# BogdanDIA/gr-dvbt

Hardware: AMD Instinct MI355X
Metric: RX Msamples/s (baseband in -> TS out) (higher is better)
Workload: dtype u8 (Viterbi/RS) + f32 (front end)

## Files before the change

gr_dvbt_amd/binding.py:

```python
import ctypes as C
import os
import subprocess
import numpy as np

_HERE = os.path.dirname(os.path.abspath(__file__))
_ROOT = os.path.dirname(_HERE)
_SO = os.path.join(_HERE, "lib", "libdvbt_hip.so")
_SRC = os.path.join(_HERE, "csrc", "dvbt_hip.hip")

QPSK, QAM16, QAM64 = 0, 1, 2
AUTO = -1
NH = 0
C1_2, C2_3, C3_4, C5_6, C7_8 = 0, 1, 2, 3, 4
T2k, T8k = 0, 1
G1_32, G1_16, G1_8, G1_4 = 0, 1, 2, 3
(TAP_ACQ, TAP_FFT, TAP_EQ, TAP_DEMAP, TAP_SYMDEINT, TAP_BITDEINT, TAP_VITERBI, TAP_DEINT, TAP_RS,
 TAP_TS, TAP_CP_START, TAP_SYMBOL_INDEX, TAP_FREQ_OFFSET, TAP_BITDEINT_LP, TAP_SOFT, TAP_CSI, TAP_BITDEINT_LOG) = range(17)
ALPHA1, ALPHA2, ALPHA4 = 1, 2, 3


class DvbtError(RuntimeError):
    pass


# ... 165 lines not shown
    def set_cut(self, stream_symbol_offset):
        cut = RxCut(int(stream_symbol_offset), 0, 0)
        _chk(self.L.dvbt_rx_set_cut(self.h, C.byref(cut)))

    def run_device(self, dptr, nsamples, stream=None):
        rep = RxReport()
        _chk(self.L.dvbt_rx_segment_run_device(self.h, C.c_void_p(dptr), nsamples, C.c_void_p(stream) if stream else None, C.byref(rep)))
        self.report = rep
        return rep

    def enqueue_device(self, dptr, nsamples, stream=None):
        _chk(self.L.dvbt_rx_segment_enqueue_device(self.h, C.c_void_p(dptr), nsamples,
                                                   C.c_void_p(stream) if stream else None))

    def finish(self):
        rep = RxReport()
        _chk(self.L.dvbt_rx_segment_finish(self.h, C.byref(rep)))
        self.report = rep
        return rep

    def tap(self, tap):
        r = self.report
        d = self.dims
        sizes = {TAP_ACQ: r.n_symbols * d.fft_length * 8, TAP_FFT: r.n_symbols * d.fft_length * 8,
                 TAP_EQ: r.n_out_symbols * d.payload_length * 8, TAP_DEMAP: r.n_out_symbols * d.payload_length,
                 TAP_SYMDEINT: r.n_out_symbols * d.payload_length, TAP_BITDEINT: r.n_out_symbols * d.payload_length,
                 TAP_VITERBI: r.n_viterbi_bytes, TAP_DEINT: r.n_rs_bytes // 188 * 204, TAP_RS: r.n_rs_bytes,
                 TAP_TS: r.n_ts_bytes, TAP_CP_START: r.n_symbols * 4, TAP_SYMBOL_INDEX: max(r.n_symbols - 1, 0) * 4,
                 TAP_FREQ_OFFSET: max(r.n_symbols - 1, 0) * 4, TAP_BITDEINT_LP: r.n_out_symbols * d.payload_length,
                 TAP_SOFT: r.n_out_symbols * d.payload_length * d.m, TAP_CSI: r.n_out_symbols * d.payload_length * 4}
        nbytes = max(int(sizes[tap]), 0)
        buf = np.zeros(nbytes, np.uint8)
        if nbytes:
            n = _chk(self.L.dvbt_rx_read_tap(self.h, tap, buf.ctypes.data_as(C.c_void_p), nbytes))
            buf = buf[:n]
        out = buf.view(self._TAP_DTYPE.get(tap, np.uint8))
        if tap in (TAP_ACQ, TAP_FFT):
            out = out.reshape(-1, d.fft_length)
        elif tap in (TAP_EQ, TAP_DEMAP, TAP_SYMDEINT, TAP_BITDEINT, TAP_BITDEINT_LP, TAP_CSI):
            out = out.reshape(-1, d.payload_length)
        elif tap == TAP_SOFT:
            out = out.reshape(-1, d.payload_length * d.m)
        return out

    def lock_periods(self):
        n = _chk(self.L.dvbt_rx_lock_periods(self.h, None, 0))
        buf = (LockPeriod * max(n, 1))()
        _chk(self.L.dvbt_rx_lock_periods(self.h, buf, n))
        return [(b.offset, b.first_call, b.cp_start0, b.n_symbols, b.first_out_symbol) for b in buf[:n]]

    def walk_stats(self):
        class W(C.Structure):
            _fields_ = [("small_passes", C.c_int64), ("general_passes", C.c_int64), ("small_chunk_calls", C.c_int32), ("small_max_calls", C.c_int32)]
        w = W()
        self.L.dvbt_rx_walk_stats.argtypes = [C.c_void_p, C.POINTER(W)]
        _chk(self.L.dvbt_rx_walk_stats(self.h, C.byref(w)))
        return w.small_passes, w.general_passes, w.small_chunk_calls, w.small_max_calls

    def period_taps(self):
        class P(C.Structure):
            _fields_ = [("bitdeint_offset", C.c_int64), ("bitdeint_bytes", C.c_int64), ("viterbi_offset", C.c_int64), ("viterbi_bytes", C.c_int64)]
        self.L.dvbt_rx_period_taps.argtypes = [C.c_void_p, C.c_void_p, C.c_int]
        n = _chk(self.L.dvbt_rx_period_taps(self.h, None, 0))
        buf = (P * max(n, 1))()
        _chk(self.L.dvbt_rx_period_taps(self.h, buf, n))
        total = max([b.bitdeint_offset + b.bitdeint_bytes for b in buf[:n]] + [0])
        log = np.zeros(total, np.uint8)
        if total:
            _chk(self.L.dvbt_rx_read_tap(self.h, TAP_BITDEINT_LOG, log.ctypes.data_as(C.c_void_p), total))
        return [(log[b.bitdeint_offset:b.bitdeint_offset + b.bitdeint_bytes], int(b.viterbi_offset), int(b.viterbi_bytes)) for b in buf[:n]]

    def viterbi_proof(self):
        p = ViterbiProof()
        self.L.dvbt_rx_viterbi_proof.argtypes = [C.c_void_p, C.POINTER(ViterbiProof)]
        _chk(self.L.dvbt_rx_viterbi_proof(self.h, C.byref(p)))
        return {"chunks": int(p.chunks), "decoded_again": int(p.decoded_again), "sequential": int(p.sequential), "not_proven": int(p.not_proven)}

    def viterbi_proof_total(self):
        p = ViterbiProof()
        self.L.dvbt_rx_viterbi_proof_total.argtypes = [C.c_void_p, C.POINTER(ViterbiProof)]
        _chk(self.L.dvbt_rx_viterbi_proof_total(self.h, C.byref(p)))
        return {"chunks": int(p.chunks), "decoded_again": int(p.decoded_again), "sequential": int(p.sequential), "not_proven": int(p.not_proven)}

    def viterbi_check(self):
        a, b = C.c_int64(), C.c_int64()
        self.L.dvbt_rx_viterbi_check.argtypes = [C.c_void_p, C.POINTER(C.c_int64), C.POINTER(C.c_int64)]
        _chk(self.L.dvbt_rx_viterbi_check(self.h, C.byref(a), C.byref(b)))
        return int(a.value), int(b.value)

    def tap_device_ptr(self, tap):
        return self.L.dvbt_rx_tap_device_ptr(self.h, tap)

    def enable_timing(self, on=True):
        _chk(self.L.dvbt_rx_enable_timing(self.h, int(on)))

    def stage_ms(self, name):
        return self.L.dvbt_rx_stage_ms(self.h, name.encode())

    def close(self):
        if self.h:
            self.L.dvbt_rx_destroy(self.h)
            self.h = C.c_void_p()

    def __del__(self):
        try:
            self.close()
        except Exception:
            pass


class StreamParams(C.Structure):
    _fields_ = [("rx", RxParams), ("segment_superframes", C.c_int), ("rank", C.c_int), ("world", C.c_int), ("ts_ring_bytes", C.c_int64), ("borrow_device_pushes", C.c_int), ("chains", C.c_int)]


class StreamInfo(C.Structure):
    _fields_ = [("status", C.c_int32), ("pieces_in_flight", C.c_int32), ("finished", C.c_int32),
                ("samples_pushed", C.c_int64), ("ts_bytes_decoded", C.c_int64), ("ts_bytes_ready", C.c_int64), ("ts_bytes_pulled", C.c_int64),
                ("first_superframe_call", C.c_int64), ("first_ts_packet", C.c_int64),
                ("constellation", C.c_int32), ("hierarchy", C.c_int32), ("code_rate", C.c_int32), ("auto_configured", C.c_int32), ("samples_released", C.c_int64), ("in_walk", C.c_int32)]


class RxStream:

    def __init__(self, constellation, code_rate, mode, segment_superframes=0, guard=G1_32, hierarchy=NH, snr_db=30.0, viterbi_bsize=768,
                 rs_oracle_compat=0, device=0, rank=0, world=0, soft_decision=0, ts_ring_bytes=0, borrow=0, viterbi_warm_windows=0, viterbi_verify=0, chains=0):
        self.L = lib()
        for fn in ("create", "push", "push_device", "finish", "status"):
            getattr(self.L, f"dvbt_rx_stream_{fn}").restype = C.c_int
        self.L.dvbt_rx_stream_create.argtypes = [C.POINTER(StreamParams), C.POINTER(C.c_void_p)]
        self.L.dvbt_rx_stream_push.argtypes = [C.c_void_p, C.c_void_p, C.c_size_t]
        self.L.dvbt_rx_stream_push_device.argtypes = [C.c_void_p, C.c_void_p, C.c_size_t, C.c_void_p]
        self.L.dvbt_rx_stream_pull.restype = C.c_int64
        self.L.dvbt_rx_stream_pull.argtypes = [C.c_void_p, C.c_void_p, C.c_size_t]
        self.L.dvbt_rx_stream_finish.argtypes = [C.c_void_p]
        self.L.dvbt_rx_stream_status.argtypes = [C.c_void_p, C.POINTER(StreamInfo)]
        self.L.dvbt_rx_stream_destroy.argtypes = [C.c_void_p]
        rx = RxParams(constellation, hierarchy, code_rate, guard, mode, 0, 0, snr_db, viterbi_bsize, rs_oracle_compat, 1, 0, device, 0, 0, 0, 0.0, soft_decision)
        rx.viterbi_warm_windows = viterbi_warm_windows
        rx.viterbi_verify = viterbi_verify
        self.p = StreamParams(rx, segment_superframes, rank, world, ts_ring_bytes, borrow, chains)
        self.L.dvbt_rx_stream_pull_chunk.restype = C.c_int64
        self.L.dvbt_rx_stream_pull_chunk.argtypes = [C.c_void_p, C.c_void_p, C.c_size_t, C.POINTER(C.c_int64)]
        self.h = C.c_void_p()
        _chk(self.L.dvbt_rx_stream_create(C.byref(self.p), C.byref(self.h)))
        self._out = np.empty(1 << 22, np.uint8)

    def push(self, iq):
        iq = np.ascontiguousarray(iq, dtype=np.complex64)
        _chk(self.L.dvbt_rx_stream_push(self.h, iq.ctypes.data_as(C.c_void_p), len(iq)))

    def push_device(self, dptr, nsamples, stream=None):
        _chk(self.L.dvbt_rx_stream_push_device(self.h, C.c_void_p(dptr), nsamples, C.c_void_p(stream) if stream else None))

    def pull(self, max_bytes=None):
        chunks = []
        left = max_bytes
        while left is None or left > 0:
            cap = len(self._out) if left is None else min(len(self._out), left)
            n = _chk(self.L.dvbt_rx_stream_pull(self.h, self._out.ctypes.data_as(C.c_void_p), cap))
            if n <= 0:
                break
            chunks.append(self._out[:n].copy())
            if left is not None:
                left -= n
        return np.concatenate(chunks) if chunks else np.zeros(0, np.uint8)

# ... 191 lines not shown
TAG_SYNC_START, TAG_SUPERFRAME_START, TAG_SYMBOL_INDEX = 1, 2, 3


class Tag(C.Structure):
    _fields_ = [("rel_offset", C.c_int64), ("key", C.c_int32), ("value", C.c_int32)]


class Sideband(C.Structure):
    _fields_ = [("in_tags", C.POINTER(Tag)), ("n_in_tags", C.c_int), ("out_tags", C.POINTER(Tag)), ("out_cap", C.c_int),
                ("n_out_tags", C.c_int), ("n_consumed", C.c_int)]


def _params(fields):
    return type("P", (C.Structure,), {"_fields_": fields})


_I = C.c_int
BLOCK_PARAMS = {
    "ofdm_sym_acquisition": _params([("blocks", _I), ("fft_length", _I), ("occupied_tones", _I), ("cp_length", _I), ("snr", C.c_float)]),
    "fft": _params([("fft_size", _I), ("forward", _I), ("shift", _I)]),
    "demod_reference_signals": _params([(n, _I) for n in ("itemsize", "ninput", "noutput", "constellation", "hierarchy", "code_rate_hp",
                                                          "code_rate_lp", "guard_interval", "transmission_mode", "include_cell_id", "cell_id")]),
    "demap": _params([("nsize", _I), ("constellation", _I), ("hierarchy", _I), ("transmission_mode", _I), ("gain", C.c_float)]),
    "symbol_inner_interleaver": _params([("nsize", _I), ("transmission_mode", _I), ("direction", _I)]),
    "bit_inner_deinterleaver": _params([("nsize", _I), ("constellation", _I), ("hierarchy", _I), ("transmission_mode", _I)]),
    "viterbi_decoder": _params([("constellation", _I), ("hierarchy", _I), ("code_rate", _I), ("bsize", _I), ("S0", _I), ("SK", _I)]),
    "convolutional_deinterleaver": _params([("blocks", _I), ("I", _I), ("M", _I)]),
    "reed_solomon_dec": _params([(n, _I) for n in ("p", "m", "gfpoly", "n", "k", "t", "s", "blocks", "oracle_compat")]),
    "energy_descramble": _params([("nblocks", _I)]),
    "resampler": _params([("interpolation", _I), ("decimation", _I), ("scale", C.c_float)]),
    "energy_dispersal": _params([("nblocks", _I)]),
    "reed_solomon_enc": _params([(n, _I) for n in ("p", "m", "gfpoly", "n", "k", "t", "s", "blocks")]),
    "convolutional_interleaver": _params([("blocks", _I), ("I", _I), ("M", _I)]),
    "inner_coder": _params([(n, _I) for n in ("ninput", "noutput", "constellation", "hierarchy", "code_rate")]),
    "bit_inner_interleaver": _params([("nsize", _I), ("constellation", _I), ("hierarchy", _I), ("transmission_mode", _I)]),
    "map": _params([("nsize", _I), ("constellation", _I), ("hierarchy", _I), ("transmission_mode", _I), ("gain", C.c_float)]),
    "reference_signals": _params([(n, _I) for n in ("itemsize", "ninput", "noutput", "constellation", "hierarchy", "code_rate_hp",
                                                    "code_rate_lp", "guard_interval", "transmission_mode", "include_cell_id", "cell_id")]),
}
TX_BLOCKS = ("energy_dispersal", "reed_solomon_enc", "convolutional_interleaver", "inner_coder", "bit_inner_interleaver", "map", "reference_signals")


class Block:

    def __init__(self, name, *args):
        self.L = lib()
        self.name = name
        self.params = BLOCK_PARAMS[name](*args)
        self.h = C.c_void_p()
        _chk(getattr(self.L, f"dvbt_{name}_create")(C.byref(self.params), C.byref(self.h)))
        self._work = getattr(self.L, f"dvbt_{name}_work")
        self._work.argtypes = [C.c_void_p, C.c_int, C.c_int, C.c_void_p, C.c_void_p, C.POINTER(Sideband)]
        self._work_device = getattr(self.L, f"dvbt_{name}_work_device", None)
        if self._work_device is not None:
            self._work_device.argtypes = [C.c_void_p, C.c_int, C.c_int, C.c_void_p, C.c_void_p, C.POINTER(Sideband), C.c_void_p]
        self._tout = (Tag * 4096)()

    def forecast(self, noutput_items):
        n = C.c_int()
        _chk(getattr(self.L, f"dvbt_{self.name}_forecast")(self.h, noutput_items, C.byref(n)))
        return n.value

    def work(self, noutput_items, ninput_items, inp, out, tags=()):
        tin = (Tag * max(len(tags), 1))(*[Tag(*t) for t in tags])
        tout = (Tag * 4096)()
        sb = Sideband(tin, len(tags), tout, 4096, 0, 0)
        r = _chk(self._work(self.h, noutput_items, ninput_items, inp.ctypes.data_as(C.c_void_p), out.ctypes.data_as(C.c_void_p), C.byref(sb)))
        return r, sb.n_consumed, [(tout[i].rel_offset, tout[i].key, tout[i].value) for i in range(min(sb.n_out_tags, 4096))]

    def work_device(self, noutput_items, ninput_items, in_ptr, out_ptr, tags=(), stream=None):
        tin = (Tag * max(len(tags), 1))(*[Tag(*t) for t in tags])
        tout = self._tout
        sb = Sideband(tin, len(tags), tout, 4096, 0, 0)
        r = _chk(self._work_device(self.h, noutput_items, ninput_items, C.c_void_p(in_ptr), C.c_void_p(out_ptr), C.byref(sb),
                                   C.c_void_p(stream) if stream else None))
        return r, sb.n_consumed, [(tout[i].rel_offset, tout[i].key, tout[i].value) for i in range(min(sb.n_out_tags, 4096))]

    def viterbi_proof(self):
        p = ViterbiProof()
        self.L.dvbt_viterbi_decoder_proof.argtypes = [C.c_void_p, C.POINTER(ViterbiProof)]
        _chk(self.L.dvbt_viterbi_decoder_proof(self.h, C.byref(p)))
        return {"chunks": int(p.chunks), "decoded_again": int(p.decoded_again), "sequential": int(p.sequential), "not_proven": int(p.not_proven)}

    def close(self):
        if self.h:
            fn = getattr(self.L, f"dvbt_{self.name}_destroy")
            fn.argtypes = [C.c_void_p]
            fn(self.h)
            self.h = C.c_void_p()

    def __del__(self):
        try:
            self.close()
        except Exception:
            pass
```

gr_dvbt_amd/csrc/dvbt_blocks.inc:

```

namespace {

struct PinBuf {
  PinMem<uint8_t> mem; void *p = nullptr; size_t cap = 0;
  int reserve(size_t n) { if (n <= cap) return DVBT_OK; p = nullptr; cap = 0; HIPCHK(mem.alloc(n + 64)); p = mem; cap = n; return DVBT_OK; }
};
struct BlockCtx {
  Stream s; DevBuf din, dout, aux; PinBuf pin_in, pin_out;
  struct Pending { void *host; size_t off, bytes; };
  std::vector<Pending> pending; size_t pin_in_used = 0, pin_out_used = 0;
  int init() { int r = need_device(); if (r) return r; HIPCHK(s.create()); return DVBT_OK; }
  static bool is_pinned(const void *host)
  {
    hipPointerAttribute_t a;
    if (hipPointerGetAttributes(&a, host) != hipSuccess) { (void)hipGetLastError(); return false; }
    return a.type == hipMemoryTypeHost;
  }
  int put(DevBuf &b, const void *host, size_t bytes, size_t offset = 0)
  {
    int r = b.reserve(offset + bytes); if (r) return r;
    if (!bytes) return DVBT_OK;
    if (is_pinned(host)) { HIPCHK(hipMemcpyAsync((char *)b.p + offset, host, bytes, hipMemcpyHostToDevice, s)); return DVBT_OK; }
    if (pin_in_used + bytes > pin_in.cap) {
      if (pin_in_used) HIPCHK(hipStreamSynchronize(s));
// ... 193 lines not shown
  return n;
}
extern "C" int dvbt_symbol_inner_interleaver_work_device(dvbt_symbol_inner_interleaver *h, int nout, int nin, const void *in, void *out, dvbt_sideband *sb, void *stream)
{
  if (!h || !in || !out) return fail(DVBT_ERR_INVALID, "null argument");
  sb_begin(sb);
  int n = nout < nin ? nout : nin; if (n <= 0) return 0;
  WCHK(sym_indices(h, n, sb));
  WCHK(sym_run(h, n, in, out, pick(stream, h->c)));
  if (sb) sb->n_consumed = n;
  return n;
}
extern "C" void dvbt_symbol_inner_interleaver_destroy(dvbt_symbol_inner_interleaver *h) { delete h; }

struct dvbt_bit_inner_deinterleaver { dvbt_bit_inner_deinterleaver_params p; BlockCtx c; Dims d; };
extern "C" int dvbt_bit_inner_deinterleaver_create(const dvbt_bit_inner_deinterleaver_params *p, dvbt_bit_inner_deinterleaver **out)
{
  BLK_CREATE_PROLOGUE(dvbt_bit_inner_deinterleaver);
  h->p = *p;
  h->d = make_dims(p->constellation, p->hierarchy, 0, 0, p->transmission_mode);
  if (!h->d.valid || p->nsize <= 0 || p->nsize % 126 || p->nsize > 49152) return fail(DVBT_ERR_INVALID, "nsize must be a positive multiple of 126");
  if (p->hierarchy != DVBT_NH && h->d.m == 2) return fail(DVBT_ERR_INVALID, "hierarchical QPSK does not exist (the reference's constructor divides by d_v - 2 = 0)");
  *out = hold.release(); return DVBT_OK;
}
extern "C" int dvbt_bit_inner_deinterleaver_forecast(const dvbt_bit_inner_deinterleaver *, int n, int *req) { if (req) *req = n; return DVBT_OK; }
static void bit_run(dvbt_bit_inner_deinterleaver *h, int n, const void *din, void *dout, hipStream_t s, void *dout_lp = nullptr)
{
  const size_t P = h->p.nsize;
  InnerParams ip; memset(&ip, 0, sizeof ip); ip.payload = (int)P; ip.m = h->d.m; ip.hier = h->p.hierarchy != DVBT_NH ? 1 : 0;
  hipLaunchKernelGGL(inner_kernel<4>, dim3(n), dim3(INNER_THREADS), inner_lds_bytes(P), s, (const float2 *)nullptr, (const uint8_t *)din, ip,
                     (const RxState *)nullptr, n, (const int *)nullptr, (const float2 *)nullptr, (const unsigned char *)nullptr,
                     (const uint16_t *)nullptr, (const uint16_t *)nullptr, (uint8_t *)nullptr, (uint8_t *)nullptr, (uint8_t *)dout, (uint8_t *)dout_lp);
}
extern "C" int dvbt_bit_inner_deinterleaver_work_hier(dvbt_bit_inner_deinterleaver *h, int nout, int nin, const void *in, void *out_hp, void *out_lp, dvbt_sideband *sb)
{
  if (!h || !in || !out_hp || !out_lp) return fail(DVBT_ERR_INVALID, "null argument");
  if (h->p.hierarchy == DVBT_NH) return fail(DVBT_ERR_STATE, "a non-hierarchical bit_inner_deinterleaver has one output");
  sb_begin(sb);
  int n = nout < nin ? nout : nin; if (n <= 0) return 0;
  size_t P = h->p.nsize;
  WCHK(h->c.put(h->c.din, in, (size_t)n * P)); WCHK(h->c.dout.reserve((size_t)n * P)); WCHK(h->c.aux.reserve((size_t)n * P));
  bit_run(h, n, h->c.din.p, h->c.dout.p, h->c.s, h->c.aux.p);
  WCHK(h->c.get(out_hp, h->c.dout.p, (size_t)n * P)); WCHK(h->c.get(out_lp, h->c.aux.p, (size_t)n * P)); WCHK(h->c.sync());
  if (sb) sb->n_consumed = n;
  return n;
}
extern "C" int dvbt_bit_inner_deinterleaver_work_hier_device(dvbt_bit_inner_deinterleaver *h, int nout, int nin, const void *in, void *out_hp, void *out_lp, dvbt_sideband *sb, void *stream)
{
  if (!h || !in || !out_hp || !out_lp) return fail(DVBT_ERR_INVALID, "null argument");
  if (h->p.hierarchy == DVBT_NH) return fail(DVBT_ERR_STATE, "a non-hierarchical bit_inner_deinterleaver has one output");
  sb_begin(sb);
  int n = nout < nin ? nout : nin; if (n <= 0) return 0;
  bit_run(h, n, in, out_hp, pick(stream, h->c), out_lp);
  if (sb) sb->n_consumed = n;
  return n;
}
extern "C" int dvbt_bit_inner_deinterleaver_work(dvbt_bit_inner_deinterleaver *h, int nout, int nin, const void *in, void *out, dvbt_sideband *sb)
{
  if (!h || !in || !out) return fail(DVBT_ERR_INVALID, "null argument");
  sb_begin(sb);
  int n = nout < nin ? nout : nin; if (n <= 0) return 0;
  size_t P = h->p.nsize;
  WCHK(h->c.put(h->c.din, in, (size_t)n * P)); WCHK(h->c.dout.reserve((size_t)n * P));
  bit_run(h, n, h->c.din.p, h->c.dout.p, h->c.s);
  WCHK(h->c.get(out, h->c.dout.p, (size_t)n * P)); WCHK(h->c.sync());
  if (sb) sb->n_consumed = n;
  return n;
}
extern "C" int dvbt_bit_inner_deinterleaver_work_device(dvbt_bit_inner_deinterleaver *h, int nout, int nin, const void *in, void *out, dvbt_sideband *sb, void *stream)
{
  if (!h || !in || !out) return fail(DVBT_ERR_INVALID, "null argument");
  sb_begin(sb);
  int n = nout < nin ? nout : nin; if (n <= 0) return 0;
  bit_run(h, n, in, out, pick(stream, h->c));
  if (sb) sb->n_consumed = n;
  return n;
}
extern "C" void dvbt_bit_inner_deinterleaver_destroy(dvbt_bit_inner_deinterleaver *h) { delete h; }

struct dvbt_viterbi_decoder {
  dvbt_viterbi_decoder_params p; BlockCtx c; Dims d; VitParams vp;
  size_t hist = 0; long long in_total = 0, steps = 0; int d_init = 0;
  static constexpr size_t kTail = 8192;
  VitProof proof; DevMem<int> carry; int cur = 0; bool have_carry = false; long long grid0 = 0;
};
extern "C" int dvbt_viterbi_decoder_create(const dvbt_viterbi_decoder_params *p, dvbt_viterbi_decoder **out)
{
  BLK_CREATE_PROLOGUE(dvbt_viterbi_decoder);
  h->p = *p;
  h->d = make_dims(p->constellation, p->hierarchy, p->code_rate, 0, 0);
  if (!h->d.valid || p->bsize <= 0 || (2 * h->d.k * p->bsize) % 16 || (p->bsize * h->d.n) % h->d.m || (p->bsize * h->d.k) % 8)
    return fail(DVBT_ERR_INVALID, "bsize must make bsize*n/m and bsize*k/8 integral and 2*k*bsize a multiple of 16");
  h->vp = make_vit_params(h->d, p->bsize, 11 * V3_BLK);
  if (h->carry.alloc(2 * V3_SLOT) != hipSuccess) return fail(DVBT_ERR_HIP, "hipMalloc (viterbi_decoder carry)");
  WCHK(h->proof.reserve(256));
  *out = hold.release(); return DVBT_OK;
}
extern "C" int dvbt_viterbi_decoder_forecast(const dvbt_viterbi_decoder *h, int n, int *req)
{ if (!h || !req) return DVBT_ERR_INVALID; *req = n * 8 * h->d.n / (h->d.k * h->d.m); return DVBT_OK; }
static int viterbi_call(dvbt_viterbi_decoder *h, int nout, int nin, const void *in, void *out, dvbt_sideband *sb, bool dev, hipStream_t s)
{
  sb_begin(sb);
  const int d_nout = h->vp.d_nbits / 16, d_nsym = h->vp.d_nsymbols;
  int nblocks = nout / d_nout;
  if (nblocks * d_nsym > nin) nblocks = nin / d_nsym;
  if (nblocks <= 0) return 0;
  const dvbt_tag *t = find_tag(sb, DVBT_TAG_SUPERFRAME_START, 0, (int64_t)nblocks * d_nsym);
  if (t) {
    h->d_init = 0; h->steps = 0; h->in_total = 0; h->hist = 0; h->have_carry = false; h->grid0 = 0;
    if (t->rel_offset > 0) { if (sb) sb->n_consumed = (int)t->rel_offset; return 0; }
    HIPCHK(hipMemsetAsync(h->proof.ctl + V3_CTL_ACC, 0, 3 * sizeof(int), s));
  }
  const size_t nbytes = (size_t)nblocks * d_nsym, hist = h->hist;
  WCHK(h->c.din.reserve_keep(dvbt_viterbi_decoder::kTail + nbytes + 64, hist, s));
  if (dev) WCHK(h->c.put_dev(h->c.din, in, nbytes, hist, s)); else { HIPCHK(hipMemcpyAsync((char *)h->c.din.p + hist, in, nbytes, hipMemcpyHostToDevice, s)); }
  const long long in_base = h->in_total - (long long)hist;
  long long out_lo = h->steps / 8 - h->d.ntb; if (out_lo < 0) out_lo = 0;
  h->steps += (long long)nblocks * (h->vp.d_nbits / 2);
  h->in_total += (long long)nbytes;
  long long out_hi = h->steps / 8 - h->d.ntb; if (out_hi < 0) out_hi = 0;
  const long long produced = out_hi - out_lo;
  if (produced > 0) {
    uint8_t *o = (uint8_t *)out;
    if (!dev) { WCHK(h->c.dout.reserve((size_t)produced)); o = (uint8_t *)h->c.dout.p; }
    const int B = h->vp.chunk_bytes;
    const long long g0 = h->have_carry ? h->grid0 : 0, chunks = (out_hi - g0 + B - 1) / B;
    if (chunks + 2 > h->proof.cap) { HIPCHK(hipStreamSynchronize(s)); int acc[3]; HIPCHK(hipMemcpy(acc, h->proof.ctl + V3_CTL_ACC, sizeof acc, hipMemcpyDeviceToHost));
                                     WCHK(h->proof.reserve(2 * chunks + 2)); HIPCHK(hipMemcpy(h->proof.ctl + V3_CTL_ACC, acc, sizeof acc, hipMemcpyHostToDevice)); }
    V3Aux ax = h->proof.aux();
    ax.grid0 = g0; ax.carry_in = h->have_carry ? h->carry + h->cur * V3_SLOT : nullptr;
    const long long b0_last = g0 + (chunks - 1) * B;
    ax.carry_rel = (int)((out_hi - b0_last) / V3_BLK) * V3_BLK; ax.carry_out = h->carry + (h->cur ^ 1) * V3_SLOT;
    launch_viterbi(s, (const uint8_t *)h->c.din.p, o, (const RxState *)nullptr, h->steps, h->vp, in_base, out_lo, produced, &ax, VIT_REPAIR);
    h->cur ^= 1; h->have_carry = true; h->grid0 = b0_last + ax.carry_rel;
    if (!dev) WCHK(h->c.get(out, h->c.dout.p, (size_t)produced));
  }
  {
    const size_t total = hist + nbytes, keep = total < dvbt_viterbi_decoder::kTail ? total : dvbt_viterbi_decoder::kTail;
    if (total > keep) {
      WCHK(h->c.aux.reserve(dvbt_viterbi_decoder::kTail));
      HIPCHK(hipMemcpyAsync(h->c.aux.p, (const char *)h->c.din.p + total - keep, keep, hipMemcpyDeviceToDevice, s));
      HIPCHK(hipMemcpyAsync(h->c.din.p, h->c.aux.p, keep, hipMemcpyDeviceToDevice, s));
    }
    h->hist = keep;
  }
  if (!dev) WCHK(h->c.sync());
  if (h->d_init == 0) { add_tag(sb, 0, DVBT_TAG_SUPERFRAME_START, 1); h->d_init = 1; }
  if (sb) sb->n_consumed = (int)nbytes;
  return (int)produced;
}
extern "C" int dvbt_viterbi_decoder_work(dvbt_viterbi_decoder *h, int nout, int nin, const void *in, void *out, dvbt_sideband *sb)
{
  if (!h || !in || !out) return fail(DVBT_ERR_INVALID, "null argument");
  return viterbi_call(h, nout, nin, in, out, sb, false, h->c.s);
}
extern "C" int dvbt_viterbi_decoder_work_device(dvbt_viterbi_decoder *h, int nout, int nin, const void *in, void *out, dvbt_sideband *sb, void *stream)
{
  if (!h || !in || !out) return fail(DVBT_ERR_INVALID, "null argument");
  return viterbi_call(h, nout, nin, in, out, sb, true, pick(stream, h->c));
}
extern "C" int dvbt_viterbi_decoder_set_warm_windows(dvbt_viterbi_decoder *h, int windows)
{
  if (!h) return fail(DVBT_ERR_INVALID, "null handle");
  if (windows == 0) windows = V3_WARM;
  if (windows < 2 * V3_BLK || windows > 576 || windows % V3_BLK != 0) return fail(DVBT_ERR_INVALID, "warm-up must be 0 (default) or a multiple of 24 in [48, 576]");
  h->vp.warm = windows;
  return DVBT_OK;
}
extern "C" int dvbt_viterbi_decoder_proof(dvbt_viterbi_decoder *h, dvbt_viterbi_proof *out)
{
  if (!h || !out) return fail(DVBT_ERR_INVALID, "null argument");
  int acc[3] = {0, 0, 0};
  HIPCHK(hipMemcpy(acc, h->proof.ctl + V3_CTL_ACC, sizeof acc, hipMemcpyDeviceToHost));
  out->chunks = acc[0]; out->decoded_again = acc[1]; out->sequential = acc[2]; out->not_proven = -1;
  return DVBT_OK;
}
extern "C" void dvbt_viterbi_decoder_destroy(dvbt_viterbi_decoder *h) { delete h; }

struct dvbt_convolutional_deinterleaver { dvbt_convolutional_deinterleaver_params p; BlockCtx c; size_t hist = 0; long long pos = 0; };
extern "C" int dvbt_convolutional_deinterleaver_create(const dvbt_convolutional_deinterleaver_params *p, dvbt_convolutional_deinterleaver **out)
{
  BLK_CREATE_PROLOGUE(dvbt_convolutional_deinterleaver);
  h->p = *p;
  if (p->I != 12 || p->M != 17 || p->blocks != 136) return fail(DVBT_ERR_INVALID, "only the DVB-T outer interleaver I=12, M=17, blocks=136 (every RX flowgraph; assert at convolutional_deinterleaver_impl.cc:68)");
  *out = hold.release(); return DVBT_OK;
}
extern "C" int dvbt_convolutional_deinterleaver_forecast(const dvbt_convolutional_deinterleaver *h, int n, int *req)
{ if (!h || !req) return DVBT_ERR_INVALID; *req = n * h->p.I * h->p.blocks; return DVBT_OK; }
static int convdeint_call(dvbt_convolutional_deinterleaver *h, int nout, int nin, const void *in, void *out, dvbt_sideband *sb, bool dev, hipStream_t s)
{
  sb_begin(sb);
  const int item = h->p.I * h->p.blocks;
  int n = nout & ~1;
  if ((long long)n * item > nin) n = (nin / item) & ~1;
  if (n <= 0) return 0;
  const dvbt_tag *t = find_tag(sb, DVBT_TAG_SUPERFRAME_START, 0, (int64_t)n * item);
  if (t && t->rel_offset > 0) { if (sb) sb->n_consumed = (int)t->rel_offset; return 0; }
  const size_t nbytes = (size_t)n * item, hist = h->hist, keep_max = 2244;
  WCHK(h->c.din.reserve_keep(keep_max + nbytes + 64, hist, s));
  if (dev) WCHK(h->c.put_dev(h->c.din, in, nbytes, hist, s)); else { HIPCHK(hipMemcpyAsync((char *)h->c.din.p + hist, in, nbytes, hipMemcpyHostToDevice, s)); }
  uint8_t *o = (uint8_t *)out;
  if (!dev) { WCHK(h->c.dout.reserve(nbytes)); o = (uint8_t *)h->c.dout.p; }
  hipLaunchKernelGGL(conv_deint_kernel, dim3(512), dim3(256), 0, s, (const uint8_t *)h->c.din.p, (long long)hist, h->pos, (long long)nbytes, o);
  if (!dev) WCHK(h->c.get(out, h->c.dout.p, nbytes));
  h->pos += (long long)nbytes;
  {
    const size_t total = hist + nbytes, keep = total < keep_max ? total : keep_max;
    if (total > keep) {
      WCHK(h->c.aux.reserve(keep_max));
      HIPCHK(hipMemcpyAsync(h->c.aux.p, (const char *)h->c.din.p + total - keep, keep, hipMemcpyDeviceToDevice, s));
      HIPCHK(hipMemcpyAsync(h->c.din.p, h->c.aux.p, keep, hipMemcpyDeviceToDevice, s));
    }
    h->hist = keep;
  }
  if (!dev) WCHK(h->c.sync());
  if (sb) sb->n_consumed = (int)nbytes;
  return n;
}
extern "C" int dvbt_convolutional_deinterleaver_work(dvbt_convolutional_deinterleaver *h, int nout, int nin, const void *in, void *out, dvbt_sideband *sb)
{
  if (!h || !in || !out) return fail(DVBT_ERR_INVALID, "null argument");
  return convdeint_call(h, nout, nin, in, out, sb, false, h->c.s);
}
extern "C" int dvbt_convolutional_deinterleaver_work_device(dvbt_convolutional_deinterleaver *h, int nout, int nin, const void *in, void *out, dvbt_sideband *sb, void *stream)
{
  if (!h || !in || !out) return fail(DVBT_ERR_INVALID, "null argument");
  return convdeint_call(h, nout, nin, in, out, sb, true, pick(stream, h->c));
}
extern "C" void dvbt_convolutional_deinterleaver_destroy(dvbt_convolutional_deinterleaver *h) { delete h; }

struct dvbt_reed_solomon_dec { dvbt_reed_solomon_dec_params p; BlockCtx c; Tables T; DevMem<int> cnt; };
extern "C" int dvbt_reed_solomon_dec_create(const dvbt_reed_solomon_dec_params *p, dvbt_reed_solomon_dec **out)
{
  BLK_CREATE_PROLOGUE(dvbt_reed_solomon_dec);
  h->p = *p;
  if (p->p != 2 || p->m != 8 || p->gfpoly != 0x11d || p->n != 255 || p->k != 239 || p->t != 8 || p->s != 51 || p->blocks <= 0)
    return fail(DVBT_ERR_INVALID, "only RS(255,239,t=8) over GF(2^8)/0x11d shortened by 51 (the DVB-T outer code)");
  WCHK(h->T.build_rs());
  if (h->cnt.alloc(2) != hipSuccess || hipMemset(h->cnt, 0, 8) != hipSuccess) return fail(DVBT_ERR_HIP, "hipMalloc");
  *out = hold.release(); return DVBT_OK;
}
extern "C" int dvbt_reed_solomon_dec_forecast(const dvbt_reed_solomon_dec *, int n, int *req) { if (req) *req = n; return DVBT_OK; }
static void rs_run(dvbt_reed_solomon_dec *h, long long words, const void *din, void *dout, hipStream_t s)
{
  hipLaunchKernelGGL(deint_rs_kernel, dim3((unsigned)((words + 63) / 64)), dim3(64), 0, s, (const uint8_t *)din, (uint8_t *)nullptr,
                     (uint8_t *)dout, (RxState *)nullptr, words, 1, 0ll, h->T.rs_tables(), h->p.oracle_compat, h->cnt, h->cnt + 1);
}
extern "C" int dvbt_reed_solomon_dec_work(dvbt_reed_solomon_dec *h, int nout, int nin, const void *in, void *out, dvbt_sideband *sb)
{
  if (!h || !in || !out) return fail(DVBT_ERR_INVALID, "null argument");
  sb_begin(sb);
  int n = nout < nin ? nout : nin; if (n <= 0) return 0;
  long long words = (long long)n * h->p.blocks;
  WCHK(h->c.put(h->c.din, in, (size_t)words * 204)); WCHK(h->c.dout.reserve((size_t)words * 188));
  rs_run(h, words, h->c.din.p, h->c.dout.p, h->c.s);
  WCHK(h->c.get(out, h->c.dout.p, (size_t)words * 188)); WCHK(h->c.sync());
  if (sb) sb->n_consumed = n;
// ... 287 lines not shown
```

gr_dvbt_amd/csrc/dvbt_hip.hip:

```cpp
#include <hip/hip_runtime.h>
#include <cstdio>
#include <cstdarg>
#include <cstdlib>
#include <cstring>
#include <string>
#include <vector>
#include <map>
#include <deque>
#include <algorithm>
#include <memory>
#include "../../include/dvbt_hip.h"
#include "hip_own.hpp"
#include "dvbt_tables.hpp"
#include "ts_ring.hpp"
#include "k_frontend.hpp"
#include "k_drift.hpp"
#include "k_backend.hpp"
#include "k_symbol8k.hpp"
#include "k_symbol2k.hpp"
#include "k_resample.hpp"
#include "k_viterbi3.hpp"
#include "k_soft4.hpp"
#include "k_quality.hpp"
#include "k_tx.hpp"
// ... 97 lines not shown
      for (size_t i = 0; i < pt.pil_k.size(); i++) pk[(size_t)s * DEMOD_NP + i] = (uint16_t)(pt.pil_k[i] | (pr[pt.pil_k[i]] < 0.f ? 0x8000 : 0));
      pli.insert(pli.end(), pt.pay_Li.begin(), pt.pay_Li.end()); pri.insert(pri.end(), pt.pay_Ri.begin(), pt.pay_Ri.end());
      pd.insert(pd.end(), pt.pay_d.begin(), pt.pay_d.end());
      for (size_t i = 0; i < pt.pay_c.size(); i++) pp.push_back((uint32_t)pt.pay_c[i] | ((uint32_t)pt.pay_Li[i] << 13) | ((uint32_t)pt.pay_d[i] << 23));
      tli.insert(tli.end(), pt.tps_Li.begin(), pt.tps_Li.end()); tri.insert(tri.end(), pt.tps_Ri.begin(), pt.tps_Ri.end());
      td.insert(td.end(), pt.tps_d.begin(), pt.tps_d.end());
      pc.insert(pc.end(), pt.pay_c.begin(), pt.pay_c.end()); pl.insert(pl.end(), pt.pay_L.begin(), pt.pay_L.end());
      prr.insert(prr.end(), pt.pay_R.begin(), pt.pay_R.end()); tl.insert(tl.end(), pt.tps_L.begin(), pt.tps_L.end());
      trr.insert(trr.end(), pt.tps_R.begin(), pt.tps_R.end());
    }
    if ((r = upload(pc, pay_c)) || (r = upload(pl, pay_L)) || (r = upload(prr, pay_R)) || (r = upload(tl, tps_L)) || (r = upload(trr, tps_R))) return r;
    if ((r = upload(pk, pil_k)) || (r = upload(pli, pay_Li)) || (r = upload(pri, pay_Ri)) || (r = upload(pd, pay_d)) || (r = upload(tli, tps_Li)) ||
        (r = upload(tri, tps_Ri)) || (r = upload(td, tps_d)) || (r = upload(pp, pay_pack))) return r;
    if ((r = upload(tps_bch_table_host(), tps_bch))) return r;
    front = true;
    return DVBT_OK;
  }
  int build_inner(float gain)
  {
    int r;
    if (!H) {
      std::vector<uint16_t> h = symbol_H(d), hi(h.size());
      for (size_t q = 0; q < h.size(); q++) hi[h[q]] = (uint16_t)q;
      if ((r = upload(h, H)) || (r = upload(hi, Hinv))) return r;
    }
    std::vector<float> p = constellation_points(d, gain);
    std::vector<float2> p2(64, make_float2(0.f, 0.f));
    for (int i = 0; i < d.csize; i++) p2[i] = make_float2(p[2 * i], p[2 * i + 1]);
    std::vector<uint8_t> lab(64, 0);
    nlev = 0; hshift = 0.f;
    if (gain > 0.f) {
      int n = 1 << (d.m / 2);
      float step = 2.0f * gain * d.norm;
      const float sh = (float)(d.alpha - 1) * gain * d.norm;
      bool ok = true;
      for (int i = 0; i < d.csize && ok; i++) {
        const float ux = p2[i].x - (p2[i].x > 0 ? sh : -sh), uy = p2[i].y - (p2[i].y > 0 ? sh : -sh);
        float fi = ux / step + 0.5f * (n - 1), fq = uy / step + 0.5f * (n - 1);
        int ii = (int)std::lround(fi), qq = (int)std::lround(fq);
        if (ii < 0 || ii >= n || qq < 0 || qq >= n || std::fabs(fi - ii) > 1e-3f || std::fabs(fq - qq) > 1e-3f) ok = false;
        else lab[ii * 8 + qq] = (uint8_t)i;
      }
      if (ok) { nlev = n; inv_step = 1.0f / step; guard = 1.0e4f * step; hshift = sh; }
    }
    if ((r = upload(p2, points)) || (r = upload(lab, label_tab))) return r;
    inner = true;
    return DVBT_OK;
  }
  InnerParams inner_params(int payload) const { InnerParams ip; ip.payload = payload; ip.m = d.m; ip.csize = d.csize; ip.nlev = nlev; ip.inv_step = inv_step; ip.guard = guard;
                                                  ip.hshift = hshift; ip.hier = d.hierarchy != 0 ? 1 : 0; return ip; }
  int build_rs()
  {
    std::vector<uint8_t> ex(512), lg(256), mul = rs_division_table();
    gf_tables(ex.data(), lg.data());
    int r;
    if ((r = upload(ex, gexp)) || (r = upload(lg, glog)) || (r = upload(mul, mul_alpha)) || (r = upload(energy_prbs(), prbs))) return r;
    rs = true;
    return DVBT_OK;
  }
  DemodTables demod_tables() const { DemodTables T; T.cpilot = cpilot; T.known_diff = known; T.tps = tps; T.pilot_ref = pref;
    T.pay_c = pay_c; T.pay_L = pay_L; T.pay_R = pay_R; T.tps_L = tps_L; T.tps_R = tps_R;
    T.pil_k = pil_k; for (int i = 0; i < 4; i++) T.np[i] = np[i];
    T.pay_Li = pay_Li; T.pay_Ri = pay_Ri; T.pay_d = pay_d; T.tps_Li = tps_Li; T.tps_Ri = tps_Ri; T.tps_d = tps_d; T.pay_pack = pay_pack; return T; }
  RsTables rs_tables() const { RsTables T; T.div_tab = mul_alpha; T.gexp = gexp; T.glog = glog; return T; }
};

#define V3_NTB_SWITCH(ntb, CALL) switch (ntb) { case 5: CALL(5); break; case 9: CALL(9); break; case 10: CALL(10); break; case 15: CALL(15); break; default: CALL(24); break; }
struct VitProof {
  DevMem<int> snap, ctl; long long cap = 0;
  int reserve(long long chunks)
  {
    if (chunks <= cap) return DVBT_OK;
    cap = 0;
    HIPCHK(snap.alloc(v3_snap_words(chunks))); HIPCHK(ctl.alloc(v3_ctl_words(chunks)));
    HIPCHK(hipMemset(ctl, 0, v3_ctl_words(chunks) * sizeof(int)));
    cap = chunks; return DVBT_OK;
  }
  V3Aux aux() const { V3Aux a; memset(&a, 0, sizeof a); a.snap = snap; a.ctl = ctl; a.cap = cap; a.carry_rel = -1; return a; }
};
enum { VIT_PLAIN = -1, VIT_REPAIR = 0, VIT_REPAIR_COUNT = 1, VIT_PROOF_ONLY = 2, VIT_FORCE_SEQ = 3, VIT_FORCE_CONFLICT = 4 };
constexpr unsigned V3_REPAIR_GRID = 64;

static void launch_viterbi(hipStream_t s, const uint8_t *in, uint8_t *out, const RxState *st, long long steps_fixed, const VitParams &vp,
                           long long in_base, long long out_lo, long long max_out_bytes, const V3Aux *ax = nullptr, int mode = VIT_PLAIN)
{
  const bool proof = ax && mode != VIT_PLAIN;
  const long long grid0 = proof ? ax->grid0 : out_lo;
  long long chunks = (out_lo + max_out_bytes - grid0 + vp.chunk_bytes - 1) / vp.chunk_bytes;
  if (chunks < 1) chunks = 1;
  const dim3 grid((unsigned)((chunks + 4 * V3_WGW - 1) / (4 * V3_WGW))), blk(64 * V3_WGW);
  V3Aux none; memset(&none, 0, sizeof none);
  if (proof) {
    V3Aux a = *ax;
    if (mode == VIT_FORCE_CONFLICT) { a.debug = 1; mode = VIT_REPAIR_COUNT; }
    const dim3 cgrid((unsigned)((chunks + 255) / 256));
    if (vp.warm == V3_WARM) {
#define V3_CALL(N) hipLaunchKernelGGL((viterbi3_kernel<N, V3_WARM, 1>), grid, blk, 0, s, in, out, st, steps_fixed, vp, a, in_base, out_lo)
      V3_NTB_SWITCH(vp.ntb, V3_CALL)
#undef V3_CALL
    } else {
#define V3_CALL(N) hipLaunchKernelGGL((viterbi3_kernel<N, 0, 1>), grid, blk, 0, s, in, out, st, steps_fixed, vp, a, in_base, out_lo)
      V3_NTB_SWITCH(vp.ntb, V3_CALL)
#undef V3_CALL
    }
    if (chunks <= V3_FIX_SMALL && mode != VIT_PROOF_ONLY) {
#define V3_CALL(N) hipLaunchKernelGGL(viterbi_fix_kernel<N>, dim3(1), blk, 0, s, in, out, st, steps_fixed, vp, a, in_base, out_lo, mode == VIT_FORCE_SEQ ? 1 : 0)
      V3_NTB_SWITCH(vp.ntb, V3_CALL)
#undef V3_CALL
      if (mode != VIT_REPAIR) {
        hipLaunchKernelGGL(viterbi_check_kernel, dim3(1), dim3(256), 0, s, a, st, steps_fixed, vp, 1);
        hipLaunchKernelGGL(viterbi_count_kernel, cgrid, dim3(256), 0, s, a, st, steps_fixed, vp);
      }
      return;
    }
    hipLaunchKernelGGL(viterbi_check_kernel, cgrid, dim3(256), 0, s, a, st, steps_fixed, vp, 0);
    if (mode == VIT_REPAIR || mode == VIT_REPAIR_COUNT) {
#define V3_CALL(N) hipLaunchKernelGGL(viterbi_repair_kernel<N>, dim3(V3_REPAIR_GRID), blk, 0, s, in, out, st, steps_fixed, vp, a, in_base, out_lo)
      V3_NTB_SWITCH(vp.ntb, V3_CALL)
#undef V3_CALL
    }
    if (mode != VIT_PROOF_ONLY) {
      const int force = mode == VIT_FORCE_SEQ ? 1 : 0;
#define V3_CALL(N) hipLaunchKernelGGL(viterbi_repair_seq_kernel<N>, dim3(1), dim3(64), 0, s, in, out, st, steps_fixed, vp, a, in_base, out_lo, force)
      V3_NTB_SWITCH(vp.ntb, V3_CALL)
#undef V3_CALL
    }
    if (mode != VIT_REPAIR) {
      hipLaunchKernelGGL(viterbi_check_kernel, dim3(1), dim3(256), 0, s, a, st, steps_fixed, vp, 1);
      hipLaunchKernelGGL(viterbi_count_kernel, cgrid, dim3(256), 0, s, a, st, steps_fixed, vp);
    }
    return;
  }
  if (vp.warm != V3_WARM) {
#define V3_CALL(N) hipLaunchKernelGGL((viterbi3_kernel<N, 0, 0>), grid, blk, 0, s, in, out, st, steps_fixed, vp, none, in_base, out_lo)
    V3_NTB_SWITCH(vp.ntb, V3_CALL)
#undef V3_CALL
    return;
  }
#define V3_CALL(N) hipLaunchKernelGGL((viterbi3_kernel<N, V3_WARM, 0>), grid, blk, 0, s, in, out, st, steps_fixed, vp, none, in_base, out_lo)
  V3_NTB_SWITCH(vp.ntb, V3_CALL)
#undef V3_CALL
}

__global__ void tail_patch_kernel(RxState *st, long long items)
{
  st->n_rs_items = items; st->n_rs_words = items * 8; st->stream_rs_items = items;
  st->rs_fail = 0; st->rs_corr = 0; st->rs_list_n = 0; st->sym_off = 0;
}

static FrontParams make_front_params(const Dims &d, float snr_db)
{
  FrontParams p; memset(&p, 0, sizeof p);
  p.N = d.N; p.cp = d.cp; p.K = d.K; p.zl = d.zl; p.payload = d.payload; p.n_cp = d.n_cp; p.n_tps = d.n_tps; p.fi_start = d.fi_start;
  p.R = ACQ_R;
  float snr = (float)pow(10, snr_db / 10.0);
  float rho = (float)(snr / (snr + 1.0));
  p.half_rho = (float)(rho / 2.0);
  return p;
}
static int set_lds(const void *fn, size_t bytes)
{
  if (bytes > 48 * 1024) HIPCHK(hipFuncSetAttribute(fn, hipFuncAttributeMaxDynamicSharedMemorySize, (int)bytes));
  return DVBT_OK;
}

enum { ST_ACQ = 0, ST_FFT, ST_DEMOD, ST_INNER, ST_VIT, ST_RS, ST_END, ST_COUNT };
static const char *kStageNames[] = {"acq", "fft", "demod", "inner", "viterbi", "rs"};

struct ResamplerDesign {
  int ri = 0, rd = 0, nt = 0; std::vector<float> taps; DevMem<float> br;
  int build(int interp, int decim)
  {
    if (interp <= 0 || decim <= 0) return fail(DVBT_ERR_INVALID, "bad resampler ratio");
    taps = resampler_taps(interp, decim, ri, rd);
    std::vector<float> b = resampler_branches(taps, ri, nt);
    if ((long long)ri * nt > RS_MAX_BRANCH_FLOATS || 256ll * rd / ri + nt + 2 > RS_TILE_IN) return fail(DVBT_ERR_INVALID, "resampler ratio outside the supported range");
    HIPCHK(br.alloc(b.size()));
    HIPCHK(hipMemcpy(br, b.data(), b.size() * sizeof(float), hipMemcpyHostToDevice));
    return DVBT_OK;
  }
};

static size_t drift_scratch_doubles(size_t C) { return C * DRIFT_SCRATCH_PER_CALL + DRIFT_SCRATCH_EXTRA; }
static void drift_carve(DriftBufs &D, double *mem, size_t C)
{
  D.tabs = mem; D.ex_run = D.tabs + C * DRIFT_TAB; D.ex_entry = D.ex_run + C; D.d = D.ex_entry + C; D.S = D.d + C; D.e = D.S + C; D.c = D.e + C; D.A0 = D.c + C;
}
static void launch_drift(hipStream_t s, const FrontParams &fp, const RxState *st, const SymMeta *meta, const DriftBufs &D, int C)
{
  hipLaunchKernelGGL(drift_prep_kernel, dim3((C + 255) / 256), dim3(256), 0, s, fp, st, meta, D);
  hipLaunchKernelGGL(drift_exact_kernel, dim3(1), dim3(1024), 0, s, fp, st, meta, D);
  const dim3 rg((C + 255) / 256);
  hipLaunchKernelGGL(drift_round_kernel<0>, rg, dim3(256), 0, s, fp, st, meta, D, (const double *)nullptr, (const double *)nullptr, D.d);
  hipLaunchKernelGGL(drift_round_kernel<1>, rg, dim3(256), 0, s, fp, st, meta, D, (const double *)D.d, (const double *)nullptr, D.e);
  hipLaunchKernelGGL(drift_round_kernel<1>, rg, dim3(256), 0, s, fp, st, meta, D, (const double *)D.e, (const double *)nullptr, D.d);
  hipLaunchKernelGGL(drift_round_kernel<2>, rg, dim3(256), 0, s, fp, st, meta, D, (const double *)D.d, (const double *)D.e, D.S);
  hipLaunchKernelGGL(drift_seq_kernel, dim3(1), dim3(64), 0, s, fp, st, meta, D);
  hipLaunchKernelGGL(drift_table_kernel, dim3(C), dim3(fp.N / 32 < 256 ? fp.N / 32 : 256), 0, s, fp, st, meta, D);
}

struct dvbt_rx {
  dvbt_rx_params prm; Dims d; Tables T; FrontParams fp; VitParams vp;
  Stream front_stream; Event front_ev[2];
  Stream own_stream; hipStream_t cur_stream = nullptr;
  Event ev[ST_COUNT];
  Stream aux_stream; Event aux_ev;
  static constexpr int NCTX = 3;
  PinMem<RxState> st_host_ctx[NCTX];
  size_t max_samples = 0; int max_calls = 0;
  DevMem<float2> d_iq;
  ResamplerDesign rsd; DevMem<float2> rs_iq; size_t chain_max = 0;
  DevMem<AcqState> acq_carry; bool use_carry = false;
  DevMem<float2> g_init; DevMem<float> l_init; DevMem<float2> g_trk; DevMem<float> l_trk;
  SymMeta *meta = nullptr; RxState *st = nullptr, *st_host = nullptr; DevMem<TpsState> tps_state;
  DevMem<RxState> st_ctx[NCTX]; DevMem<SymMeta> meta_ctx[NCTX]; int ctx = 0;
  DevMem<int> trk_flags_ctx[NCTX], sym_ticket_ctx[NCTX], drift_flags_ctx[NCTX];
  DevMem<int> trk_cp_a, trk_cp_b; int *trk_flags = nullptr; DevMem<float> trk_eps; DevMem<TpsEdge> tps_edges;
  DevMem<int> centre, anchor_pos;
  DevMem<float2> acq_tap, fft_out, eq, tpsval; DevMem<SymInfo> info; DevMem<int> maj, sym_index;
  DevMem<uint8_t> labels, symdeint_tap, bitdeint, vit, deint_tap, rs_out, ts_out;
  DevMem<uint8_t> bitdeint_lp;
  DevMem<float2> q_sym; DevMem<double> q_mer; DevMem<unsigned long long> q_cnt;
  unsigned long long seg_serial = 0, q_eq_serial = 0;
  DevMem<uint8_t> bd_log; std::vector<dvbt_period_tap> plog; size_t plog_bytes = 0;
  VitProof vproof; bool vit_checked = false;
  size_t vit_cap = 0; DevMem<RsDefer> rs_defer; int rs_defer_cap = 0;
  DevMem<unsigned long long> rs_sync;
  unsigned soft_grid = 0;
  DevMem<float> csi; DevMem<int8_t> soft_a; DevMem<uint16_t> soft_tab; DevMem<unsigned> soft_scratch;
  int timing = 0;
  bool pending = false;
  double acc_ms[ST_COUNT] = {0}; long n_timed = 0; bool ev_recorded = false;
  dvbt_rx_report last; bool have_last = false;
  dvbt_rx_cut cut = {0, 0, 0};
  DevMem<float2> tps_prev, tps_prev_snap[2]; DevMem<TpsState> tps_snap[2]; DevMem<DescrRun> descr_runs; DevMem<int> descr_nruns;
  int descr_runs_cap = 0;
  int n_periods = 1; size_t seg_offset = 0;
  std::vector<dvbt_lock_period> periods;
  DriftBufs drift = {nullptr, nullptr, nullptr, nullptr, nullptr, nullptr, nullptr, nullptr, nullptr, nullptr}; DevMem<double> drift_mem; DevMem<float> drift_delta;
  struct GraphEntry { const void *iq; size_t n; hipStream_t s; long long sym_off; int delay, phase; hipGraphExec_t exec; };
  std::vector<GraphEntry> graphs;
  int ncu = 256;
  long long n_small = 0, n_general = 0;
  int sym_grid = 512;
  int *sym_ticket = nullptr;
  ~dvbt_rx();
};

constexpr long long kVitMaxChunk = 3000;
static int vit_chunk_bytes(const dvbt_rx *h, long long max_vit);

static void drop_graphs(dvbt_rx *h)
{
  for (auto &ge : h->graphs) if (ge.exec) (void)hipGraphExecDestroy(ge.exec);
  h->graphs.clear();
}
dvbt_rx::~dvbt_rx() { drop_graphs(this); }

extern "C" int dvbt_rx_create(const dvbt_rx_params *p, dvbt_rx **out)
{
  if (!p || !out) return fail(DVBT_ERR_INVALID, "null argument");
  int r = need_device(); if (r) return r;
  Dims d = make_dims(p->constellation, p->hierarchy, p->code_rate, p->guard_interval, p->transmission_mode);
  if (!d.valid) return fail(DVBT_ERR_INVALID, "bad DVB-T parameters");
  if (p->viterbi_bsize <= 0 || (2 * d.k * p->viterbi_bsize) % 16 != 0 || (p->viterbi_bsize * d.n) % d.m != 0)
    return fail(DVBT_ERR_INVALID, "viterbi_bsize must make bsize*n/m integral and 2*k*bsize a multiple of 16");
  if (d.hierarchy != 0 && d.m == 2) return fail(DVBT_ERR_INVALID, "hierarchical QPSK does not exist (the reference's bit_inner_deinterleaver divides by d_v - 2 = 0 in its constructor)");
  if (d.hierarchy != 0 && p->soft_decision) return fail(DVBT_ERR_INVALID, "soft decisions are built for the non-hierarchical modes");
  if (p->hier_stream < 0 || p->hier_stream > 1) return fail(DVBT_ERR_INVALID, "hier_stream must be 0 (HP) or 1 (LP)");
  if (p->viterbi_warm_windows != 0 && (p->viterbi_warm_windows < 2 * V3_BLK || p->viterbi_warm_windows > V3_WARM_MAX || p->viterbi_warm_windows % V3_BLK != 0))
    return fail(DVBT_ERR_INVALID, "viterbi_warm_windows must be 0 (default) or a multiple of 24 in [48, 1152]");
  if (p->viterbi_warm_windows != 0 && p->soft_decision) return fail(DVBT_ERR_INVALID, "viterbi_warm_windows applies to the hard-decision decoder");
  if (p->viterbi_verify < VIT_PLAIN || p->viterbi_verify > VIT_FORCE_CONFLICT) return fail(DVBT_ERR_INVALID, "viterbi_verify must lie in [-1, 4]");
  if (p->viterbi_verify > 0 && p->soft_decision) return fail(DVBT_ERR_INVALID, "viterbi_verify applies to the hard-decision decoder");
  HIPCHK(hipSetDevice(p->device));
  std::unique_ptr<dvbt_rx> hold(new dvbt_rx()); dvbt_rx *const h = hold.get();
  h->prm = *p; h->d = d; h->T.d = d;
  size_t chain_max = p->max_samples;
  if (p->resample_interp != 0 || p->resample_decim != 0) {
    if ((r = h->rsd.build(p->resample_interp, p->resample_decim))) return r;
    chain_max = (size_t)(((unsigned long long)p->max_samples * h->rsd.ri + h->rsd.rd - 1) / h->rsd.rd);
  }
  if (chain_max < (size_t)(2 * d.N + d.cp + 16)) return fail(DVBT_ERR_INVALID, "max_samples smaller than one acquisition window");
  h->chain_max = chain_max;
  h->fp = make_front_params(d, p->snr_db);
  int cb = p->viterbi_chunk_bytes > 0 ? p->viterbi_chunk_bytes : 768;
  h->vp = make_vit_params(d, p->viterbi_bsize, cb);
  if (p->viterbi_warm_windows > 0) h->vp.warm = p->viterbi_warm_windows;
  h->max_samples = p->max_samples;
  h->max_calls = (int)((chain_max - (2 * d.N + d.cp + 16)) / (d.N + d.cp) + 1);
  if ((r = h->T.build_fft(d.N)) || (r = h->T.build_front()) || (r = h->T.build_inner(1.0f)) || (r = h->T.build_rs())) return r;
  HIPCHK(h->own_stream.create());
  if (p->front_priority) {
    int least = 0, greatest = 0; HIPCHK(hipDeviceGetStreamPriorityRange(&least, &greatest));
    HIPCHK(h->front_stream.create(hipStreamNonBlocking, greatest));
    for (int i = 0; i < 2; i++) HIPCHK(h->front_ev[i].create(hipEventDisableTiming));
  }
  if (h->rsd.ri) HIPCHK(h->rs_iq.alloc(chain_max + 16));
  const size_t C = (size_t)h->max_calls, N = d.N, P = d.payload;
  HIPCHK(h->g_init.alloc(ACQ_INIT_TRIES_MAX * N)); HIPCHK(h->l_init.alloc(ACQ_INIT_TRIES_MAX * N));
  HIPCHK(h->g_trk.alloc(C * 2 * ACQ_R)); HIPCHK(h->l_trk.alloc(C * 2 * ACQ_R));
  for (int i = 0; i < dvbt_rx::NCTX; i++) { HIPCHK(h->meta_ctx[i].alloc(C)); HIPCHK(h->st_ctx[i].alloc(1)); HIPCHK(hipMemset(h->st_ctx[i], 0, sizeof(RxState))); }
  h->meta = h->meta_ctx[0]; h->st = h->st_ctx[0]; h->ctx = 0;
  HIPCHK(h->trk_cp_a.alloc(C)); HIPCHK(h->trk_cp_b.alloc(C));
  HIPCHK(h->trk_eps.alloc(C));
  for (int i = 0; i < dvbt_rx::NCTX; i++) { HIPCHK(h->trk_flags_ctx[i].alloc(16)); HIPCHK(hipMemset(h->trk_flags_ctx[i], 0, sizeof(int) * 16)); }
  h->trk_flags = h->trk_flags_ctx[0];
// ... 254 lines not shown
  const long long cut_sym_off = o.cut_set ? o.sym_off : (long long)h->cut.stream_symbol_offset;
  const int cut_delay = o.cut_set ? o.delay : h->cut.start_delay_symbols;
  cut_hunt(fp, d, cut_delay);
  fp.ncalls = (int)((nsamples - (2 * d.N + d.cp + 16)) / (d.N + d.cp) + 1);
  fp.hist = o.hist; fp.keep_last = o.keep_last ? 1 : 0; fp.avail = o.avail > 0 ? o.avail : (long long)nsamples;
  const int C = fp.ncalls, N = d.N;
  h->cur_stream = s;
  hipStream_t const s_user = s;
  const bool split = h->front_stream && !o.acq_only && !o.skip_acq && !o.continuation && h->timing != 1 && C >= 512 && !h->prm.launch_graph;
  if (split) { HIPCHK(hipEventRecord(h->front_ev[0], s_user)); HIPCHK(hipStreamWaitEvent(h->front_stream, h->front_ev[0], 0)); s = h->front_stream; }
  auto join_front = [&]() -> int { if (split && s != s_user) { HIPCHK(hipEventRecord(h->front_ev[1], s)); s = s_user; HIPCHK(hipStreamWaitEvent(s, h->front_ev[1], 0)); } return DVBT_OK; };
  const bool tm = h->timing == 1 && !o.acq_only, tmv = h->timing != 0 && !o.acq_only;
  if (tm) HIPCHK(hipEventRecord(h->ev[ST_ACQ], s));
  if (o.skip_acq) {
    if (!o.continuation && !o.tps_init) HIPCHK(reset_tps_state(h, s));
  } else {
  const AcqState *carry = nullptr;
  int tries = C < o.init_tries ? C : o.init_tries;
  hipLaunchKernelGGL(acq_metric_kernel, dim3((N + 255) / 256, tries), dim3(256), 0, s, iq, fp, (const RxState *)h->st, 0, h->g_init, h->l_init, 0);
  const AcqReset rz = {h->trk_flags, h->sym_ticket, (o.acq_only || o.continuation || o.tps_init) ? nullptr : reinterpret_cast<int *>(h->tps_state.get()),(int)(sizeof(TpsState) / 4),
                       o.carry_avg, o.use_carry ? 1 : 0};
  hipLaunchKernelGGL(acq_init_fsm_kernel, dim3(1), dim3(1024), (size_t)N * 5, s, fp, h->st, (const float2 *)h->g_init, (const float *)h->l_init, carry, 0, tries, rz);
  if (o.acq_only && !o.no_small && C <= ACQ_SMALL_MAX_CALLS) {
    const int cpc = acq_small_cpc(d.cp);
    h->n_small++;
    hipLaunchKernelGGL(acq_small_kernel, dim3(1), dim3(64 * (1 + cpc / 2)), (size_t)cpc * 2 * (d.cp + 2 * ACQ_R) * sizeof(float2), s, iq, fp, h->st, h->meta, cpc, h->drift.flags);
  } else {
  if (o.acq_only) h->n_general++;
  {
    const int n_anchors = (C - 1) / ACQ_ANCHOR;
    if (n_anchors > 0) hipLaunchKernelGGL(acq_anchor_kernel, dim3(n_anchors), dim3(1024), acq_anchor_lds_bytes(N, d.cp), s, iq, fp, (const RxState *)h->st, h->anchor_pos);
    hipLaunchKernelGGL(acq_centre_kernel, dim3((C + 1023) / 1024), dim3(1024), 0, s, fp, (const RxState *)h->st, (const int *)h->anchor_pos, n_anchors, h->centre);
  }
  hipLaunchKernelGGL(acq_track_metric_kernel, dim3((C + ACQ_TM_CALLS - 1) / ACQ_TM_CALLS), dim3(256), 0, s, iq, fp, (const RxState *)h->st, (const int *)h->centre, h->g_trk, h->l_trk);
  constexpr int kIters = TRK_ROUNDS;
  hipLaunchKernelGGL(acq_track_fused_kernel, dim3((C + TRK_OWN - 1) / TRK_OWN), dim3(256), 0, s, fp, (const RxState *)h->st, (const float2 *)h->g_trk,
                     (const float *)h->l_trk, h->trk_cp_a, h->trk_eps, h->trk_flags, (const int *)h->centre);
  hipLaunchKernelGGL(acq_finalize_kernel, dim3((C + 1023) / 1024), dim3(1024), 0, s, fp, h->st, (const int *)h->trk_cp_a, (const float *)h->trk_eps,
                     (const int *)h->trk_flags, kIters - 1, h->meta, h->trk_flags + kIters, (const float *)h->l_trk, (const int *)h->centre);
  hipLaunchKernelGGL(acq_track_light_kernel, dim3(1), dim3(64), 0, s, fp, h->st, (const float2 *)h->g_trk, (const float *)h->l_trk, h->meta,
                     (const int *)(h->trk_flags + kIters), h->trk_flags + kIters + 1, (const int *)h->centre, iq);
  hipLaunchKernelGGL(acq_track_kernel, dim3(1), dim3(64), 0, s, fp, h->st, (const float2 *)h->g_trk, (const float *)h->l_trk, h->meta,
                     (const int *)(h->trk_flags + kIters + 1), (AcqState *)nullptr, (const int *)h->centre, iq);
  }
  if (o.acq_only) {
    HIPCHK(hipMemcpyAsync(h->st_host, h->st, sizeof(RxState), hipMemcpyDeviceToHost, s));
    HIPCHK(hipGetLastError());
    return DVBT_OK;
  }
  }
  if (tm) HIPCHK(hipEventRecord(h->ev[ST_FFT], s));
  const bool drift_off = o.skip_acq && h->st_host->drift_known_off;
  if (!drift_off) {
    launch_drift(s, fp, h->st, h->meta, h->drift, C);
  }
  launch_symbols(h, s, iq, fp, C, drift_off);
  if (tm) HIPCHK(hipEventRecord(h->ev[ST_DEMOD], s));
  long long max_vit = (long long)C * d.payload * d.m * d.k / (8 * d.n) + 1;
  if (o.vit_off + (size_t)max_vit > h->vit_cap) return fail(DVBT_ERR_CAPACITY, "Viterbi stream buffer too small for the segment's lock periods");
  { int r = launch_frames(h, s, fp, C, o.continuation, o.tps_init, cut_sym_off, tm ? (hipEvent_t)h->ev[ST_INNER] : nullptr); if (r) return r; }
  InnerParams ip = h->T.inner_params(d.payload);
  if (h->prm.soft_decision) {
    const float step = 2.0f * d.norm;
    hipLaunchKernelGGL(soft_demap_kernel, dim3(C), dim3(256), (size_t)d.payload * d.m, s, (const float2 *)h->eq, (const float *)h->csi, (const RxState *)h->st, ip, (const float2 *)h->T.points,
                       1.0f / (step * step), (const int *)h->sym_index, (const uint16_t *)h->soft_tab, h->soft_a);
    { int r = join_front(); if (r) return r; }
    if (tmv) HIPCHK(hipEventRecord(h->ev[ST_VIT], s));
    const S4Plan sp = s4_plan(max_vit, d.ntb);
    const unsigned grid = std::min(s4_grid(max_vit, d.ntb), h->soft_grid);
    hipLaunchKernelGGL(viterbi_soft4_kernel, dim3(grid), dim3(64 * S4_WAVES), 0, s, (const int8_t *)h->soft_a, h->vit + o.vit_off, (const RxState *)h->st, h->vp,
                       h->soft_scratch, sp.B, sp.nsteps);
  } else {
  { int r = join_front(); if (r) return r; }
  if (tmv) HIPCHK(hipEventRecord(h->ev[ST_VIT], s));
  VitParams vp = h->vp;
  vp.chunk_bytes = vit_chunk_bytes(h, max_vit);
  const bool proof = h->vproof.snap && h->prm.viterbi_verify != VIT_PLAIN;
  V3Aux ax = h->vproof.aux();
  if (proof) {
    if (max_vit / vp.chunk_bytes + 2 > h->vproof.cap) return fail(DVBT_ERR_CAPACITY, "Viterbi proof: state buffer too small for this segment's chunks");
    h->vit_checked = true;
  }
  launch_viterbi(s, (const uint8_t *)((h->prm.hier_stream && h->bitdeint_lp) ? h->bitdeint_lp : h->bitdeint), h->vit + o.vit_off, (const RxState *)h->st, 0ll, vp, 0ll, 0ll, max_vit,
                 proof ? &ax : nullptr, h->prm.viterbi_verify);
  }
  if (tmv) HIPCHK(hipEventRecord(h->ev[ST_RS], s));
  if (o.tail) { int r = enqueue_tail(h, s, max_vit / 204 + 1, -1); if (r) return r; }
  if (tm) HIPCHK(hipEventRecord(h->ev[ST_END], s));
  if (tmv) h->ev_recorded = true;
  HIPCHK(hipMemcpyAsync(h->st_host, h->st, sizeof(RxState), hipMemcpyDeviceToHost, s));
  HIPCHK(hipGetLastError());
  h->pending = true;
  return DVBT_OK;
}

extern "C" int dvbt_rx_segment_enqueue_device(dvbt_rx *h, const void *iq_device, size_t nsamples, void *stream)
{
  if (!h || !iq_device) return fail(DVBT_ERR_INVALID, "null argument");
  HIPCHK(hipSetDevice(h->prm.device));
  hipStream_t s = stream ? (hipStream_t)stream : h->own_stream;
  const float2 *chain; size_t chain_n;
  int r = prepare_chain(h, (const float2 *)iq_device, nsamples, s, &chain, &chain_n); if (r) return r;
  h->n_periods = 1; h->seg_offset = 0;
  if (h->prm.launch_graph && !h->timing && !h->rsd.ri && !(h->acq_tap || h->fft_out || h->symdeint_tap || h->deint_tap)) {
    for (auto &ge : h->graphs)
      if (ge.iq == chain && ge.n == chain_n && ge.s == s && ge.sym_off == h->cut.stream_symbol_offset && ge.delay == h->cut.start_delay_symbols && ge.phase == h->cut.descr_call_phase) {
        HIPCHK(hipGraphLaunch(ge.exec, s));
        h->cur_stream = s; h->pending = true;
        return DVBT_OK;
      }
    if (h->graphs.size() < 16) {
      hipGraph_t gr = nullptr; hipGraphExec_t ex = nullptr;
      HIPCHK(hipStreamBeginCapture(s, hipStreamCaptureModeThreadLocal));
      const int r = enqueue(h, chain, chain_n, s);
      const hipError_t e = hipStreamEndCapture(s, &gr);
      if (r) { if (gr) (void)hipGraphDestroy(gr); return r; }
      if (e != hipSuccess || !gr) return fail(DVBT_ERR_HIP, std::string("hipStreamEndCapture: ") + hipGetErrorString(e));
      const hipError_t e2 = hipGraphInstantiate(&ex, gr, nullptr, nullptr, 0);
      (void)hipGraphDestroy(gr);
      if (e2 != hipSuccess) return fail(DVBT_ERR_HIP, std::string("hipGraphInstantiate: ") + hipGetErrorString(e2));
      h->graphs.push_back(dvbt_rx::GraphEntry{chain, chain_n, s, (long long)h->cut.stream_symbol_offset, h->cut.start_delay_symbols, h->cut.descr_call_phase, ex});
      HIPCHK(hipGraphLaunch(ex, s));
      h->cur_stream = s; h->pending = true;
      return DVBT_OK;
    }
  }
  return enqueue(h, chain, chain_n, s);
}

static void fill_report(dvbt_rx *h, const RxState &s, dvbt_rx_report &r)
{
  memset(&r, 0, sizeof r);
  r.status = s.status; r.n_symbols = s.n_symbols; r.first_out_symbol = s.first_out; r.n_out_symbols = s.n_out_symbols;
  r.cp_start0 = s.cp_start0; r.first_call = s.call0;
  r.resume_sample = ((s.status & 2) && !(s.status & 1)) ? (int64_t)(s.call0 + s.n_symbols) * (h->d.N + h->d.cp) + (h->d.N + h->d.cp) / 2 : 0;
  r.n_viterbi_bytes = s.n_vit_bytes; r.n_rs_items = s.n_rs_items; r.n_rs_bytes = s.n_rs_words * 188;
  r.n_ts_bytes = s.n_ts_bytes; r.rs_fail_words = s.rs_fail; r.rs_corrected_symbols = s.rs_corr;
  r.stream_symbol_offset = s.sym_off; r.ts_first_packet = s.ts_first_packet; r.stream_rs_items = s.stream_rs_items;
  r.tps_valid = (int32_t)(s.tps_bits >> 63); r.tps_bits = s.tps_bits & ~(1ull << 63);
  if (r.tps_valid) {
    auto fld = [&](int first, int last) { int v = 0; for (int i = first; i <= last; i++) v = (v << 1) | (int)((s.tps_bits >> i) & 1ull); return v; };
    r.tps_length_indicator = fld(17, 22); r.tps_constellation = fld(25, 26); r.tps_hierarchy = fld(27, 29);
    r.tps_code_rate_hp = fld(30, 32); r.tps_code_rate_lp = fld(33, 35); r.tps_guard_interval = fld(36, 37);
    r.tps_transmission_mode = fld(38, 39); r.tps_cell_id = fld(40, 47);
    const dvbt_rx_params &q = h->prm;
    r.tps_mismatch = (r.tps_constellation != q.constellation ? 1 : 0) | (r.tps_hierarchy != q.hierarchy ? 2 : 0) | (r.tps_code_rate_hp != q.code_rate ? 4 : 0) |
                     (r.tps_guard_interval != q.guard_interval ? 8 : 0) | (r.tps_transmission_mode != q.transmission_mode ? 16 : 0);
    if (r.tps_mismatch) r.status |= 16;
  }
}

extern "C" int dvbt_rx_segment_finish(dvbt_rx *h, dvbt_rx_report *rep)
{
  if (!h) return fail(DVBT_ERR_INVALID, "null handle");
  if (!h->pending) return fail(DVBT_ERR_STATE, "no segment enqueued");
  HIPCHK(hipStreamSynchronize(h->cur_stream));
  h->pending = false;
  if (h->timing && h->ev_recorded) {
    for (int i = h->timing == 2 ? ST_VIT : 0; i < (h->timing == 2 ? ST_RS : ST_END); i++) { float ms = 0; if (hipEventElapsedTime(&ms, h->ev[i], h->ev[i + 1]) == hipSuccess) h->acc_ms[i] += ms; }
    float ms = 0; if (h->timing == 1 && hipEventElapsedTime(&ms, h->ev[0], h->ev[ST_END]) == hipSuccess) h->acc_ms[ST_END] += ms;
    h->n_timed++; h->ev_recorded = false;
  }
  dvbt_rx_report r;
  fill_report(h, *h->st_host, r);
  r.n_lock_periods = r.first_out_symbol >= 0 ? 1 : 0;
  h->last = r; h->have_last = true; h->seg_serial++;
  if (rep) *rep = r;
// ... 419 lines not shown
  const dvbt_rx_report &r = h->last; const Dims &d = h->d;
  size_t ns = r.n_symbols > 0 ? (size_t)r.n_symbols : 0, no = r.n_out_symbols > 0 ? (size_t)r.n_out_symbols : 0;
  size_t fo = r.first_out_symbol > 0 ? (size_t)r.first_out_symbol : 0;
  switch (tap) {
    case DVBT_TAP_ACQ: *ptr = h->acq_tap; *bytes = ns * d.N * 8; break;
    case DVBT_TAP_FFT: *ptr = h->fft_out; *bytes = ns * d.N * 8; break;
    case DVBT_TAP_EQ: *ptr = h->eq ? (void *)(h->eq + fo * d.payload) : nullptr; *bytes = no * d.payload * 8; break;
    case DVBT_TAP_DEMAP: *ptr = h->labels ? (void *)(h->labels + fo * d.payload) : nullptr; *bytes = no * d.payload; break;
    case DVBT_TAP_SYMDEINT: *ptr = h->symdeint_tap; *bytes = no * d.payload; break;
    case DVBT_TAP_BITDEINT: *ptr = h->bitdeint; *bytes = no * d.payload; break;
    case DVBT_TAP_VITERBI: *ptr = h->vit; *bytes = (size_t)r.n_viterbi_bytes; break;
    case DVBT_TAP_DEINT: *ptr = h->deint_tap; *bytes = (size_t)(r.n_rs_bytes / 188) * 204; break;
    case DVBT_TAP_RS: *ptr = h->rs_out; *bytes = (size_t)r.n_rs_bytes; break;
    case DVBT_TAP_TS: *ptr = h->ts_out; *bytes = (size_t)r.n_ts_bytes; break;
    case DVBT_TAP_SYMBOL_INDEX: *ptr = h->sym_index; *bytes = (ns > 0 ? ns - 1 : 0) * 4; break;
    case DVBT_TAP_BITDEINT_LOG: *ptr = h->bd_log; *bytes = h->plog_bytes; break;
    case DVBT_TAP_BITDEINT_LP: *ptr = h->bitdeint_lp; *bytes = no * d.payload; break;
    case DVBT_TAP_SOFT: *ptr = h->soft_a; *bytes = no * d.payload * d.m; break;
    case DVBT_TAP_CSI: *ptr = h->csi ? (void *)(h->csi + fo * d.payload) : nullptr; *bytes = no * d.payload * 4; break;
    default: return fail(DVBT_ERR_INVALID, "unknown tap");
  }
  return DVBT_OK;
}

extern "C" int64_t dvbt_rx_read_tap(dvbt_rx *h, int tap, void *dst, size_t cap)
{
  if (!h || !dst) return fail(DVBT_ERR_INVALID, "null argument");
  if (tap == DVBT_TAP_CP_START) {
    size_t ns = h->have_last && h->last.n_symbols > 0 ? (size_t)h->last.n_symbols : 0;
    std::vector<SymMeta> m(ns);
    if (ns) HIPCHK(hipMemcpy(m.data(), h->meta, ns * sizeof(SymMeta), hipMemcpyDeviceToHost));
    size_t n = ns * 4 <= cap ? ns : cap / 4;
    for (size_t i = 0; i < n; i++) ((int32_t *)dst)[i] = m[i].cp_start;
    return (int64_t)(n * 4);
  }
  if (tap == DVBT_TAP_FREQ_OFFSET) {
    size_t ns = h->have_last && h->last.n_symbols > 1 ? (size_t)h->last.n_symbols - 1 : 0;
    std::vector<SymInfo> m(ns);
    if (ns) HIPCHK(hipMemcpy(m.data(), h->info, ns * sizeof(SymInfo), hipMemcpyDeviceToHost));
    size_t n = ns * 4 <= cap ? ns : cap / 4;
    for (size_t i = 0; i < n; i++) ((int32_t *)dst)[i] = m[i].freq_offset;
    return (int64_t)(n * 4);
  }
  void *p = nullptr; size_t bytes = 0;
  int r = tap_info(h, tap, &p, &bytes); if (r) return r;
  if (!p) return fail(DVBT_ERR_STATE, "tap not enabled (call dvbt_rx_enable_taps before the segment)");
  if (bytes > cap) bytes = cap;
  if (bytes) HIPCHK(hipMemcpy(dst, p, bytes, hipMemcpyDeviceToHost));
  return (int64_t)bytes;
}

extern "C" void *dvbt_rx_tap_device_ptr(dvbt_rx *h, int tap)
{
  if (!h) return nullptr;
  switch (tap) {
    case DVBT_TAP_RS: return h->rs_out; case DVBT_TAP_TS: return h->ts_out; case DVBT_TAP_VITERBI: return h->vit;
    case DVBT_TAP_FFT: return h->fft_out; case DVBT_TAP_EQ: return h->eq; case DVBT_TAP_BITDEINT: return h->bitdeint;
    default: return nullptr;
  }
}

extern "C" int dvbt_rx_viterbi_proof(dvbt_rx *h, dvbt_viterbi_proof *out)
{
  if (!h || !out) return fail(DVBT_ERR_INVALID, "null argument");
  if (!h->vproof.ctl) return fail(DVBT_ERR_STATE, "dvbt_rx_viterbi_proof: the handle runs the plain chunk decoders (viterbi_verify = -1, or soft decisions)");
  if (h->pending) return fail(DVBT_ERR_STATE, "dvbt_rx_viterbi_proof: a segment is in flight (dvbt_rx_segment_finish first)");
  HIPCHK(hipSetDevice(h->prm.device));
  int r[V3_CTL_HDR]; memset(r, 0, sizeof r); r[V3_CTL_UNPROVEN] = -1;
  if (h->vit_checked) HIPCHK(hipMemcpy(r, h->vproof.ctl, sizeof r, hipMemcpyDeviceToHost));
  out->chunks = r[V3_CTL_CHUNKS]; out->decoded_again = r[V3_CTL_MISMATCH]; out->sequential = r[V3_CTL_SEQ]; out->not_proven = r[V3_CTL_UNPROVEN];
  return DVBT_OK;
}
extern "C" int dvbt_rx_viterbi_proof_total(dvbt_rx *h, dvbt_viterbi_proof *out)
{
  if (!h || !out) return fail(DVBT_ERR_INVALID, "null argument");
  if (!h->vproof.ctl) return fail(DVBT_ERR_STATE, "dvbt_rx_viterbi_proof_total: the handle runs the plain chunk decoders (viterbi_verify = -1, or soft decisions)");
  if (h->pending) return fail(DVBT_ERR_STATE, "dvbt_rx_viterbi_proof_total: a segment is in flight (dvbt_rx_segment_finish first)");
  HIPCHK(hipSetDevice(h->prm.device));
  int acc[3] = {0, 0, 0};
  HIPCHK(hipMemcpy(acc, h->vproof.ctl + V3_CTL_ACC, sizeof acc, hipMemcpyDeviceToHost));
  out->chunks = acc[0]; out->decoded_again = acc[1]; out->sequential = acc[2]; out->not_proven = -1;
  return DVBT_OK;
}
extern "C" int dvbt_rx_viterbi_check(dvbt_rx *h, int64_t *chunks, int64_t *unproven)
{
  if (!h || !chunks || !unproven) return fail(DVBT_ERR_INVALID, "null argument");
  if (h->prm.viterbi_verify < VIT_REPAIR_COUNT) return fail(DVBT_ERR_STATE, "dvbt_rx_viterbi_check: the handle was created without the final check (viterbi_verify >= 1)");
  dvbt_viterbi_proof p; int r = dvbt_rx_viterbi_proof(h, &p); if (r) return r;
  *chunks = p.chunks; *unproven = p.not_proven < 0 ? 0 : p.not_proven;
  return DVBT_OK;
}

extern "C" int dvbt_rx_period_taps(dvbt_rx *h, dvbt_period_tap *out, int cap)
{
  if (!h) return fail(DVBT_ERR_INVALID, "null handle");
  if (!h->bd_log) return fail(DVBT_ERR_STATE, "dvbt_rx_period_taps: dvbt_rx_enable_taps(h, 2) before the segment");
  int n = 0;
  for (const dvbt_period_tap &e : h->plog) if (e.bitdeint_bytes > 0) { if (out && n < cap) out[n] = e; n++; }
  return n;
}

extern "C" int dvbt_rx_lock_periods(dvbt_rx *h, dvbt_lock_period *out, int cap)
{
  if (!h) return fail(DVBT_ERR_INVALID, "null handle");
  const int n = (int)h->periods.size();
  for (int i = 0; i < n && i < cap && out; i++) out[i] = h->periods[i];
  return n;
}

extern "C" int dvbt_rx_walk_stats(dvbt_rx *h, dvbt_walk_stats *out)
{
  if (!h || !out) return fail(DVBT_ERR_INVALID, "null argument");
  out->small_passes = h->n_small; out->general_passes = h->n_general; out->small_chunk_calls = acq_small_cpc(h->d.cp); out->small_max_calls = ACQ_SMALL_MAX_CALLS;
  return DVBT_OK;
}

extern "C" double dvbt_rx_stage_ms(dvbt_rx *h, const char *stage)
{
  if (!h || !stage || h->n_timed == 0) return -1.0;
  if (!strcmp(stage, "total")) return h->timing == 2 ? -1.0 : h->acc_ms[ST_END] / h->n_timed;
  for (int i = 0; i < ST_END; i++) if (!strcmp(stage, kStageNames[i])) return (h->timing == 2 && i != ST_VIT) ? -1.0 : h->acc_ms[i] / h->n_timed;
  return -1.0;
}

extern "C" void dvbt_rx_destroy(dvbt_rx *h) { delete h; }

extern "C" int dvbt_debug_peak_detect(const float *lam_host, const float *avg_host, int n, int32_t *out_host, float *avg_out_host)
{
  if (!lam_host || !avg_host || !out_host || !avg_out_host || n <= 0) return fail(DVBT_ERR_INVALID, "null argument");
  int r = need_device(); if (r) return r;
  DevMem<float> dl, da, dao; DevMem<int> dout;
  HIPCHK(dl.alloc((size_t)16 * n)); HIPCHK(da.alloc(n)); HIPCHK(dao.alloc((size_t)2 * n)); HIPCHK(dout.alloc((size_t)4 * n));
  HIPCHK(hipMemcpy(dl, lam_host, sizeof(float) * 16 * n, hipMemcpyHostToDevice)); HIPCHK(hipMemcpy(da, avg_host, sizeof(float) * n, hipMemcpyHostToDevice));
  hipLaunchKernelGGL(peak_selftest_kernel, dim3(n), dim3(64), 0, nullptr, (const float *)dl, (const float *)da, n, dout, dao);
  HIPCHK(hipMemcpy(out_host, dout, sizeof(int) * 4 * n, hipMemcpyDeviceToHost)); HIPCHK(hipMemcpy(avg_out_host, dao, sizeof(float) * 2 * n, hipMemcpyDeviceToHost));
  return DVBT_OK;
}

extern "C" int dvbt_debug_soft_viterbi(int constellation, int code_rate, const int8_t *soft_host, int64_t n_soft, int64_t total_steps, int B, int nsteps, int grid,
                                       uint8_t *out_host, size_t out_cap)
{
  if (!soft_host || !out_host) return fail(DVBT_ERR_INVALID, "null argument");
  const Dims d = make_dims(constellation, 0, code_rate, 0, 0);
  if (!d.valid) return fail(DVBT_ERR_INVALID, "bad DVB-T parameters");
  if (n_soft < 0 || n_soft % d.m != 0 || n_soft > (1ll << 30)) return fail(DVBT_ERR_INVALID, "n_soft must be a multiple of the constellation's m in [0, 2^30]");
  if (total_steps < 0 || total_steps > (1ll << 30)) return fail(DVBT_ERR_INVALID, "total_steps must lie in [0, 2^30]");
  if (B < 64 || B > S4_BMAX) return fail(DVBT_ERR_INVALID, "B must lie in [64, 304]");
  const int look = 8 * d.ntb > S4_LOOK ? 8 * d.ntb : S4_LOOK;
  if (nsteps <= 0 || nsteps % S4_BLK != 0 || nsteps > S4_MAXSTEPS || nsteps < S4_WARM + 8 * B + look)
    return fail(DVBT_ERR_INVALID, "nsteps must be a multiple of 48 in [256 + 8 B + max(8 ntraceback, 128), S4_MAXSTEPS]");
  if (grid < 1 || grid > S4_GRID) return fail(DVBT_ERR_INVALID, "grid must lie in [1, 2048]");
  if (out_cap == 0 || out_cap > (1ull << 30) || (long long)out_cap < total_steps / 8) return fail(DVBT_ERR_INVALID, "out_cap must hold total_steps / 8 bytes");
  int r = need_device(); if (r) return r;
  const VitParams vp = make_vit_params(d, 768, 768);
  RxState st; memset(&st, 0, sizeof st);
  st.first_out = 0; st.n_vit_steps = total_steps; st.n_vit_in = n_soft / d.m;
  DevMem<int8_t> dsoft; DevMem<uint8_t> dout; DevMem<RxState> dst; DevMem<unsigned> scratch;
  HIPCHK(dsoft.alloc((size_t)n_soft + 64)); HIPCHK(dout.alloc(out_cap)); HIPCHK(dst.alloc(1));
  HIPCHK(scratch.alloc((size_t)grid * S4_WAVES * S4_SLOT_WORDS));
  if (n_soft) HIPCHK(hipMemcpy(dsoft, soft_host, (size_t)n_soft, hipMemcpyHostToDevice));
  HIPCHK(hipMemcpy(dst, &st, sizeof st, hipMemcpyHostToDevice));
  HIPCHK(hipMemset(dout, 0xA5, out_cap));
  hipLaunchKernelGGL(viterbi_soft4_kernel, dim3((unsigned)grid), dim3(64 * S4_WAVES), 0, nullptr, (const int8_t *)dsoft, dout, (const RxState *)dst, vp, scratch, B, nsteps);
  HIPCHK(hipGetLastError());
  HIPCHK(hipMemcpy(out_host, dout, out_cap, hipMemcpyDeviceToHost));
  return DVBT_OK;
// ... 286 lines not shown
```

gr_dvbt_amd/csrc/k_viterbi3.hpp:

```cpp
#pragma once
#include <hip/hip_runtime.h>
#include <stdint.h>
#include <limits.h>
#include <string.h>
#include "dvbt_tables.hpp"
#include "k_backend.hpp"

namespace dvbt {

inline VitParams make_vit_params(const Dims &d, int bsize, int chunk_bytes)
{
  VitParams v; memset(&v, 0, sizeof v);
  v.m = d.m; v.k = d.k; v.n = d.n; v.plen = d.plen; v.ntb = d.ntb; v.bsize = bsize;
  v.d_nsymbols = bsize * d.n / d.m; v.d_nbits = 2 * d.k * bsize;
  v.chunk_bytes = chunk_bytes > 0 ? chunk_bytes : 768; v.payload = d.payload; v.warm = 72;
  memcpy(v.punct, d.punct, 16); memcpy(v.prefix, d.prefix, 16);
  v.punct_mask = 0; v.prefix_nib = 0;
  for (int i = 0; i < d.plen; i++) { v.punct_mask |= (unsigned)d.punct[i] << i; v.prefix_nib |= (unsigned long long)d.prefix[i] << (4 * i); }
  v.magic_plen = ~0ull / (unsigned)d.plen + 1; v.magic_m = ~0ull / (unsigned)d.m + 1;
  for (int i = 0; i < 64; i++) v.punct_rep |= (unsigned long long)d.punct[i % d.plen] << i;
  v.magic16_plen = (65536u + (unsigned)d.plen - 1) / (unsigned)d.plen;
  return v;
}

// ... 155 lines not shown
    asm("v_bfi_b32 %0, %1, %2, %3" : "=v"(T.z[q]) : "s"(V3_RMASK<NW>), "v"(T.wsh[q]), "v"(t[q]));
  }
}
template <int NW> __device__ __forceinline__ void v3_hop(V3Trace &T, const unsigned char *tab) { unsigned t[2]; v3_hop_read(T, tab, t); v3_hop_merge<NW>(T, t); }
__device__ __forceinline__ void v3_trace_read(const V3Trace &T, const unsigned char *tab, unsigned (&t)[2])
{
#pragma unroll
  for (int q = 0; q < 2; q++) t[q] = tab[T.z[q]];
}
template <bool MASKED> __device__ __forceinline__ void v3_trace_store(const V3Trace &T, const unsigned (&t)[2], uint8_t *outb)
{
#pragma unroll
  for (int q = 0; q < 2; q++) {
    const unsigned zz = (t[q] ^ (((t[q] >> 4) & 1u) * 12u)) & 63u;
    unsigned by = (((zz | (zz << 6)) >> T.osh[q]) & 0xfcu) | (t[q] >> 6);
    if (MASKED) {
      unsigned long long sv;
      asm volatile("s_and_saveexec_b64 %0, %1\n\tglobal_store_byte %2, %3, off\n\ts_mov_b64 exec, %0" : "=&s"(sv) : "s"(T.ok[q]), "v"(outb + T.ob[q]), "v"(by) : "memory", "scc");
    } else if ((T.ok[q] >> (threadIdx.x & 63)) & 1) outb[T.ob[q]] = (unsigned char)by;
  }
}
__device__ __forceinline__ void v3_trace_out(const V3Trace &T, const unsigned char *tab, uint8_t *outb) { unsigned t[2]; v3_trace_read(T, tab, t); v3_trace_store<false>(T, t, outb); }

__device__ __forceinline__ void v3_load_words(const unsigned *wp_, unsigned (&W)[8])
{
  const uint4 *wp = reinterpret_cast<const uint4 *>(wp_);
  const uint4 t0 = wp[0], t1 = wp[1];
  W[0] = t0.x; W[1] = t0.y; W[2] = t0.z; W[3] = t0.w; W[4] = t1.x; W[5] = t1.y; W[6] = t1.z; W[7] = t1.w;
}
template <int V6, bool HOPS, int HOP0, int NTB, int NW, bool PREF> __device__ __forceinline__ void v3_fwd_window(int (&v)[2], const V3Lane &L, const unsigned *wrow, unsigned char *tab, unsigned char *tabw,
                                                                                           unsigned char *bests, int j0, int dd, int pl, V3Trace &T, unsigned (&W)[8], unsigned (&Wn)[8], uint8_t *outb)
{
  constexpr bool HOPA = HOPS && HOP0 + 2 * V6 < NTB - 1, HOPB = HOPS && HOP0 + 2 * V6 + 1 < NTB - 1;
  constexpr bool FINA = HOPS && HOP0 + 2 * V6 == NTB - 1, FINB = HOPS && HOP0 + 2 * V6 + 1 == NTB - 1;
  unsigned th[2], tout[2];
  if (HOPA) v3_hop_read(T, tab, th);
  if (FINA) v3_trace_read(T, tab, tout);
  const int jr = (j0 + V6) & (V3_RINGW - 1);
#if V3_EXP & 256
  for (int i = 0; i < 8; i++) { W[i] = (unsigned)(j0 * 0x01010101 + i * 0x00020406 + pl); asm volatile("" : "+v"(W[i])); }
#else
  if (PREF) v3_load_words(wrow + (V6 + 1) * 8, Wn);
#endif
  constexpr int P0 = (8 * V6) % 6;
  int raw[2];
#if V3_EXP & 32
  if (V6 & 1) __builtin_amdgcn_s_setprio(1); else __builtin_amdgcn_s_setprio(0);
#endif
#if V3_EXP & 128
  __builtin_amdgcn_s_sleep(1);
#endif
  v3_step<(P0 + 0) % 6, 0>(v, W[0], L, raw); V3_YIELD(); v3_step<(P0 + 1) % 6, 0>(v, W[1], L, raw); V3_YIELD(); v3_step<(P0 + 2) % 6, 3>(v, W[2], L, raw); V3_YIELD();
  if (HOPA) { v3_hop_merge<NW>(T, th); if (HOPB) v3_hop_read(T, tab, th); }
  if (FINB) v3_trace_read(T, tab, tout);
  if (FINA) v3_trace_store<true>(T, tout, outb);
  v3_step<(P0 + 3) % 6, 0>(v, W[3], L, raw); V3_YIELD(); v3_step<(P0 + 4) % 6, 0>(v, W[4], L, raw); V3_YIELD(); v3_step<(P0 + 5) % 6, 1>(v, W[5], L, raw); V3_YIELD();
  v3_step<(P0 + 6) % 6, 4>(v, W[6], L, raw); V3_YIELD(); v3_step<(P0 + 7) % 6, 2>(v, W[7], L, raw);
  if (HOPB) v3_hop_merge<NW>(T, th);
  if (FINB) v3_trace_store<true>(T, tout, outb);
  if (!(V3_EXP & 4)) *reinterpret_cast<unsigned *>(tabw + jr * V3_ROW<NW>) = __builtin_amdgcn_perm((unsigned)raw[1], (unsigned)raw[0], 0x06040200u);
  if (V3_EXP & 2) { if (raw[0] == 0x12345) bests[jr] = 1; return; }
  const int s = v3_window_end<(P0 + 2) % 6, (V6 & 1) == 1>(v, L);
  bests[dd * V3_RINGW + jr] = (unsigned char)s;
}
template <bool HOPS, int HOP0, int NTB, int NW, bool MORE> __device__ __forceinline__ void v3_fwd_six(int (&v)[2], const V3Lane &L, const unsigned *wrow, unsigned char *tab, unsigned char *tabw,
                                                                                  unsigned char *bests, int j0, int dd, int pl, V3Trace &T, unsigned (&Wa)[8], unsigned (&Wb)[8], uint8_t *outb)
{
  v3_fwd_window<0, HOPS, HOP0, NTB, NW, true>(v, L, wrow, tab, tabw, bests, j0, dd, pl, T, Wa, Wb, outb); v3_fwd_window<1, HOPS, HOP0, NTB, NW, true>(v, L, wrow, tab, tabw, bests, j0, dd, pl, T, Wb, Wa, outb);
  v3_fwd_window<2, HOPS, HOP0, NTB, NW, true>(v, L, wrow, tab, tabw, bests, j0, dd, pl, T, Wa, Wb, outb); v3_fwd_window<3, HOPS, HOP0, NTB, NW, true>(v, L, wrow, tab, tabw, bests, j0, dd, pl, T, Wb, Wa, outb);
  v3_fwd_window<4, HOPS, HOP0, NTB, NW, true>(v, L, wrow, tab, tabw, bests, j0, dd, pl, T, Wa, Wb, outb); v3_fwd_window<5, HOPS, HOP0, NTB, NW, MORE>(v, L, wrow, tab, tabw, bests, j0, dd, pl, T, Wb, Wa, outb);
}

#if V3_EXP & 16
__device__ unsigned long long *v3_dbg;
#endif

constexpr int V3_SLOT = 32;
constexpr int V3_CTL_CHUNKS = 0;
constexpr int V3_CTL_MISMATCH = 1;
constexpr int V3_CTL_CONFLICT = 2;
constexpr int V3_CTL_UNPROVEN = 3;
constexpr int V3_CTL_SEQ = 4;
constexpr int V3_CTL_ACC = 8;
constexpr int V3_CTL_HDR = 16;
struct V3Aux {
  int *snap;
  int *ctl;
  long long cap;
  long long grid0;
  const int *carry_in;
  int *carry_out; int carry_rel;
  int debug;
};
__device__ __forceinline__ int *v3_own(const V3Aux &ax, long long c) { return ax.snap + (3 * c) * V3_SLOT; }
__device__ __forceinline__ int *v3_pred(const V3Aux &ax, long long c) { return ax.snap + (3 * c + 1) * V3_SLOT; }
__device__ __forceinline__ int *v3_fix(const V3Aux &ax, long long c) { return ax.snap + (3 * c + 2) * V3_SLOT; }
inline size_t v3_snap_words(long long cap) { return (size_t)(cap + 2) * 3 * V3_SLOT; }
inline size_t v3_ctl_words(long long cap) { return (size_t)V3_CTL_HDR + 2 * (size_t)(cap + 2); }

struct V3Lds { unsigned char *tab; unsigned *wbuf; unsigned char *bests; const unsigned *lut; int wv; };
__device__ __forceinline__ void v3_init_lut(unsigned *lut, int lane)
{
  if (lane < 16) {
    const int k0 = (lane >> 2) & 1, k1 = (lane >> 3) & 1, t1 = (lane >> 1) & 1, t0 = lane & 1;
    const int u0 = k0 ? 1 - 2 * t1 : 0, u1 = k1 ? 1 - 2 * (k0 ? t0 : t1) : 0;
    const unsigned d0 = (unsigned)(2 * (u0 + u1)) & 0xff, d1 = (unsigned)(2 * (-u0 + u1)) & 0xff;
    const unsigned d2 = (unsigned)(2 * (u0 - u1)) & 0xff, d3 = (unsigned)(2 * (-u0 - u1)) & 0xff;
    lut[lane] = d0 | (d1 << 8) | (d2 << 16) | (d3 << 24);
  }
}

template <int NTB, int WARM, int MODE, int NW>
__device__ __forceinline__ void v3_decode(const uint8_t *__restrict__ in, uint8_t *__restrict__ out, long long total_steps, long long total_out, const VitParams &vp,
                                          long long in_base, long long out_lo, long long b0, bool dec_active, const V3Lds &S, const V3Lane &L, int (&v)[2], int (&endv)[2],
                                          int *own, int *predn, const int *inject, int *carry, int carry_rel)
{
  unsigned char *const tab = S.tab; unsigned *const wbuf = S.wbuf; unsigned char *const bests = S.bests; const unsigned *const lut = S.lut;
  unsigned *const cbits = wbuf;
  constexpr int V3_CBS = V3_BLK * 8;
  static_assert(V3_CBW <= V3_CBS, "bit stream does not fit the step-word row");
  const int lane = threadIdx.x & 63, dd = lane >> 4, pl = lane & 15;
  const int rowl = S.wv * 256 + dd * 64;
  unsigned char *const tabw = tab + rowl + pl * 4;
  const int B = vp.chunk_bytes, m = vp.m;
  constexpr int ntb = NTB;
  const long long b1 = (b0 + B < total_out) ? b0 + B : total_out;
  const int warm = MODE == 2 ? 0 : WARM > 0 ? WARM : vp.warm;
  const long long w0 = b0 + 2 - warm;
  const int J = ((warm + B + ntb - 1 + V3_BLK - 1) / V3_BLK) * V3_BLK;
  const long long n_in_bytes = (total_steps * 2 / vp.plen * vp.n + vp.m - 1) / vp.m;
  const int nload = ((384 + 2 * m - 2) / m + 3 + 15) / 16;

  uint8_t *const outb = out + (b0 - out_lo);
  const int ob_end = !dec_active ? INT_MIN : (int)(b1 - b0 > INT_MIN / 2 ? b1 - b0 : INT_MIN / 2);
  const int ob_lo = MODE != 1 || out_lo <= b0 ? 0 : (int)(out_lo - b0 < INT_MAX / 2 ? out_lo - b0 : INT_MAX / 2);
  const long long tb0 = 8 * (w0 - 1) - 2;
  constexpr int BLKBITS = 2 * 8 * V3_BLK;
  const int inc_q = BLKBITS / vp.plen, inc_ph = BLKBITS - inc_q * vp.plen;
  const unsigned magic16_m = (65536u + (unsigned)m - 1) / (unsigned)m;

  int u_first, u_last;
  {
    const long long r = total_steps - 8 * V3_BLK - tb0;
    int first = tb0 >= 0 ? 0 : (int)((-tb0 + 7) >> 3 < J ? (-tb0 + 7) >> 3 : J), last = !dec_active || r < 0 ? -1 : (int)(r >> 3 < J ? r >> 3 : J);
    u_first = max(max(__builtin_amdgcn_readlane(first, 0), __builtin_amdgcn_readlane(first, 16)), max(__builtin_amdgcn_readlane(first, 32), __builtin_amdgcn_readlane(first, 48)));
    u_last = min(min(__builtin_amdgcn_readlane(last, 0), __builtin_amdgcn_readlane(last, 16)), min(__builtin_amdgcn_readlane(last, 32), __builtin_amdgcn_readlane(last, 48)));
  }
  auto pfx = [&](int ph) { return (int)__popc(vp.punct_mask & ((1u << ph) - 1u)); };
  int ph0 = 0, pf0 = 0, bo0 = 0, off = 0; long long byte0 = 0; uint4 q = make_uint4(0, 0, 0, 0);
  auto stage_load = [&](int jb) {
    const long long tb = tb0 + (long long)jb * 8;
    if (jb > 0 && jb - V3_BLK >= u_first) {
      const int pf_old = pf0;
      ph0 += inc_ph;
      const int wrap = ph0 >= vp.plen ? 1 : 0;
      ph0 -= wrap ? vp.plen : 0;
      pf0 = pfx(ph0);
      const int r = bo0 + (inc_q + wrap) * vp.n + pf0 - pf_old;
      const int dby = (int)(((unsigned)r * magic16_m) >> 16);
      bo0 = r - dby * m; byte0 += dby;
    } else {
      const unsigned long long pbit = 2ull * (unsigned long long)(tb > 0 ? tb : 0);
      const unsigned long long pq = __umul64hi(pbit, vp.magic_plen);
      ph0 = (int)(pbit - pq * (unsigned)vp.plen); pf0 = pfx(ph0);
      const unsigned long long rb = pq * (unsigned)vp.n + (unsigned)pf0;
      const unsigned long long by = __umul64hi(rb, vp.magic_m);
      byte0 = (long long)by; bo0 = (int)(rb - by * (unsigned)m);
    }
    off = (int)(((unsigned long long)(uintptr_t)in + (unsigned long long)(byte0 - in_base)) & 3ull);
    const long long src = byte0 - off + pl * 16;
    q = make_uint4(0, 0, 0, 0);
    if (dec_active && pl < nload) {
      if (src >= in_base && src + 16 <= n_in_bytes) q = *reinterpret_cast<const uint4 *>(in + (src - in_base));
      else {
        unsigned w[4] = {0, 0, 0, 0};
        for (int i = 0; i < 16; i++) {
          const long long bb = src + i;
          const unsigned bv = (bb >= in_base && bb < n_in_bytes) ? in[bb - in_base] : 0;
          w[i >> 2] |= bv << (8 * (i & 3));
        }
        q = make_uint4(w[0], w[1], w[2], w[3]);
      }
    }
  };
  auto stage_words = [&](int jb) {
    {
      const unsigned mk = (1u << m) - 1;
      auto grp = [&](unsigned d) { return ((d & mk) << (3 * m)) | (((d >> 8) & mk) << (2 * m)) | (((d >> 16) & mk) << m) | ((d >> 24) & mk); };
      const unsigned g0 = grp(q.x), g1 = grp(q.y), g2 = grp(q.z), g3 = grp(q.w);
      unsigned *cb = cbits + dd * V3_CBS;
      if (pl < nload) {
        if (m == 2) cb[pl] = (g0 << 24) | (g1 << 16) | (g2 << 8) | g3;
        else if (m == 4) { cb[2 * pl] = (g0 << 16) | g1; cb[2 * pl + 1] = (g2 << 16) | g3; }
        else { cb[3 * pl] = (g0 << 8) | (g1 >> 16); cb[3 * pl + 1] = (g1 << 16) | (g2 >> 8); cb[3 * pl + 2] = (g2 << 24) | g3; }
      }
    }
    __builtin_amdgcn_fence(__ATOMIC_SEQ_CST, "wavefront");
    constexpr int SPL = V3_BLK * 8 / 16;
    const long long tb = tb0 + (long long)jb * 8;
    const int ub0 = pl * SPL;
    int lo = 0, hi = SPL;
    int x = ph0 + 2 * ub0;
    if (jb < u_first || jb > u_last) {
      const long long tbr = tb > 0 ? tb : 0;
      const long long t = tb + ub0;
      if (t < 0) lo = (-t < SPL) ? (int)(-t) : SPL;
      const long long rem = total_steps - t;
      hi = !dec_active ? 0 : rem <= 0 ? 0 : rem < SPL ? (int)rem : SPL;
      if (hi < lo) hi = lo;
      x = ph0 + 2 * (int)((t + lo) - tbr);
      if (x < 0) x = 0;
    }
    const int dq = (int)(((unsigned)x * vp.magic16_plen) >> 16);
    const int ph = x - dq * vp.plen;
    const int pos = off * m + bo0 + dq * vp.n + pfx(ph) - pf0;
    const unsigned kmask = ((unsigned)(vp.punct_rep >> ph) << (2 * lo)) & (((1u << (2 * hi)) - 1u) & ~((1u << (2 * lo)) - 1u));
    const unsigned *cb = cbits + dd * V3_CBS;
    const unsigned cw0 = cb[pos >> 5], cw1 = cb[(pos >> 5) + 1];
    unsigned win = (unsigned)(((((unsigned long long)cw0) << 32) | cw1) >> (32 - (pos & 31)));
    unsigned idx[SPL], sw[SPL];
#pragma unroll
    for (int i = 0; i < SPL; i++) {
      const unsigned k2 = (kmask >> (2 * i)) & 3u;
      idx[i] = (k2 << 2) | (win >> 30);
      win <<= __popc(k2);
    }
#pragma unroll
    for (int i = 0; i < SPL; i++) sw[i] = lut[idx[i]];
    static_assert(SPL % 4 == 0, "a lane's step words are whole 16-byte groups (its offset dd * 768 + pl * 48 bytes is 16-byte aligned)");
    uint4 *const wdst = reinterpret_cast<uint4 *>(wbuf + dd * (V3_BLK * 8) + ub0);
#pragma unroll
    for (int i = 0; i < SPL / 4; i++) wdst[i] = make_uint4(sw[4 * i], sw[4 * i + 1], sw[4 * i + 2], sw[4 * i + 3]);
    __builtin_amdgcn_fence(__ATOMIC_SEQ_CST, "wavefront");
  };
  V3Trace T;
  int tsh[2];
#pragma unroll
  for (int c = 0; c < 2; c++) {
    T.oend[c] = c * 16 + pl < V3_BLK ? ob_end : INT_MIN; tsh[c] = (2 * ((c * 16 + pl + 1) % 3) + 4) % 6; T.osh[c] = (6 - 2 * ((c * 16 + pl + 3 * ntb - (ntb - 1)) % 3)) % 6;
  }
  static_assert(V3_BLK % 3 == 0, "phases per lane");
  auto bests_read = [&](int jp, unsigned (&bb)[2]) {
#pragma unroll
    for (int c = 0; c < 2; c++) bb[c] = bests[dd * V3_RINGW + ((jp + c * 16 + pl) & (V3_RINGW - 1))];
  };
  auto trace_init = [&](int jp, const unsigned (&bb)[2]) {
#pragma unroll
    for (int c = 0; c < 2; c++) {
      const int jj = jp + c * 16 + pl;
      T.ob[c] = jj - (warm + ntb - 1);
      T.ok[c] = __builtin_amdgcn_ballot_w64(T.ob[c] >= ob_lo && T.ob[c] < T.oend[c]);
      T.wsh[c] = jj * V3_ROW<NW> + rowl;
      const unsigned R = (bb[c] | (bb[c] << 6)) >> tsh[c];
      T.z[c] = (int)((R ^ 51u ^ (((R >> 4) & 1u) * 12u)) & 63u) | (T.wsh[c] & V3_RMASK<NW>);
    }
  };
  unsigned bb[2];

  stage_load(0);
  for (int jb = 0; jb < J; jb += V3_BLK) {
    if (MODE == 1 && dec_active) {
      if (jb == warm) { if (inject) { v[0] = inject[0]; v[1] = inject[1]; } own[0] = v[0]; own[1] = v[1]; }
      if (jb == warm + B) { predn[0] = v[0]; predn[1] = v[1]; }
      if (carry && jb == warm + carry_rel) { carry[0] = v[0]; carry[1] = v[1]; }
    }
    if (MODE == 2) {
      if (jb == 0 && dec_active) { own[0] = v[0]; own[1] = v[1]; }
      if (jb == B) { endv[0] = v[0]; endv[1] = v[1]; }
      if (carry && dec_active && jb == carry_rel) { carry[0] = v[0]; carry[1] = v[1]; }
    }
    bests_read(jb - V3_BLK, bb);
    if (!(V3_EXP & 8) || jb == 0) stage_words(jb);
    if (jb + V3_BLK < J && !(V3_EXP & 8)) stage_load(jb + V3_BLK);
    const bool tr = jb > 0 && !(V3_EXP & 1);
    if (tr) trace_init(jb - V3_BLK, bb);
    const unsigned *wrow = wbuf + dd * (V3_BLK * 8);
    unsigned Wa[8], Wb[8];
    v3_load_words(wrow, Wa);
    if (tr) {
      v3_fwd_six<true, 0, NTB, NW, true>(v, L, wrow, tab, tabw, bests, jb, dd, pl, T, Wa, Wb, outb);
      v3_fwd_six<true, 12, NTB, NW, true>(v, L, wrow + 48, tab, tabw, bests, jb + 6, dd, pl, T, Wa, Wb, outb);
    } else {
      v3_fwd_six<false, 0, NTB, NW, true>(v, L, wrow, tab, tabw, bests, jb, dd, pl, T, Wa, Wb, outb);
      v3_fwd_six<false, 0, NTB, NW, true>(v, L, wrow + 48, tab, tabw, bests, jb + 6, dd, pl, T, Wa, Wb, outb);
    }
    static_assert(V3_BLK == 24, "the second half of the block is written out: two groups of six windows, straight-line like the first half");
    static_assert(NTB - 1 < 24, "the chains' last read takes a hop slot of the first twelve windows");
    v3_fwd_six<false, 0, NTB, NW, true>(v, L, wrow + 96, tab, tabw, bests, jb + 12, dd, pl, T, Wa, Wb, outb);
    v3_fwd_six<false, 0, NTB, NW, false>(v, L, wrow + 144, tab, tabw, bests, jb + 18, dd, pl, T, Wa, Wb, outb);
  }
  __builtin_amdgcn_fence(__ATOMIC_SEQ_CST, "wavefront");
  bests_read(J - V3_BLK, bb);
  trace_init(J - V3_BLK, bb);
  for (int h = 0; h < ntb - 1; h++) v3_hop<NW>(T, tab);
  v3_trace_out(T, tab, outb);
}

template <int NW> struct V3Shared {
  alignas(16) unsigned char tab[V3_RINGW * V3_ROW<NW>];
  alignas(16) unsigned wbuf[NW][4 * V3_BLK * 8];
  unsigned char bests[NW][4 * V3_RINGW];
  unsigned lut[16];
};
static_assert(sizeof(V3Shared<4>) <= 81920 && V3_RMASK<4> == 0xffc0 && V3_RMASK<1> == 0x3fc0, "two four-wave workgroups per CU beside the symbol kernel's 76 KB");
#define V3_LDS_DECL(NW) __shared__ V3Shared<NW> sh_;
#define V3_LDS(NW, wv) V3Lds{sh_.tab, sh_.wbuf[wv], sh_.bests[wv], sh_.lut, wv}

template <int NTB, int WARM = V3_WARM, int MODE = 0> __global__ __launch_bounds__(64 * V3_WGW) void viterbi3_kernel(const uint8_t *__restrict__ in, uint8_t *__restrict__ out, const RxState *st,
                                                      long long steps_fixed, VitParams vp, V3Aux ax, long long in_base, long long out_lo)
{
  V3_LDS_DECL(V3_WGW)
  const int wv = V3_WGW > 1 ? (int)(threadIdx.x >> 6) : 0;
  const V3Lds S = V3_LDS(V3_WGW, wv);
  const int lane = threadIdx.x & 63, dd = lane >> 4, pl = lane & 15;
  const long long total_steps = st ? st->n_vit_steps : steps_fixed;
  const long long total_out = total_steps / 8 - vp.ntb;
  const int B = vp.chunk_bytes;
  if (MODE == 1 && blockIdx.x == 0 && threadIdx.x == 0) {
    ax.ctl[V3_CTL_MISMATCH] = 0; ax.ctl[V3_CTL_CONFLICT] = 0; ax.ctl[V3_CTL_UNPROVEN] = -1; ax.ctl[V3_CTL_SEQ] = 0;
  }
  const long long grid0 = MODE == 1 ? ax.grid0 : out_lo;
  const long long chunk0 = ((long long)blockIdx.x * V3_WGW + wv) * 4;
  if (grid0 + chunk0 * B >= total_out) return;
  const long long c = chunk0 + dd, b0 = grid0 + c * B;
  const bool dec_active = b0 < total_out;
  v3_init_lut(sh_.lut, lane);
#if V3_EXP & 16
  const unsigned long long dbg_t0 = wall_clock64();
#endif
  V3Lane L; v3_init_lane(pl, L);
  int v[2] = {L.arm_org[0][0], L.arm_org[0][1]}, endv[2];
  int *own = nullptr, *predn = nullptr, *carry = nullptr; const int *inject = nullptr;
  if (MODE == 1) {
    own = v3_own(ax, c) + 2 * pl; predn = v3_pred(ax, c + 1) + 2 * pl;
    if (c == 0 && ax.carry_in) inject = ax.carry_in + 2 * pl;
    if (ax.carry_out && b0 + B >= total_out) carry = ax.carry_out + 2 * pl;
  }
  v3_decode<NTB, WARM, MODE, V3_WGW>(in, out, total_steps, total_out, vp, in_base, out_lo, b0, dec_active, S, L, v, endv, own, predn, inject, carry, ax.carry_rel);
#if V3_EXP & 16
  if (lane == 0) {
    unsigned id, xcc;
    asm volatile("s_getreg_b32 %0, hwreg(HW_REG_HW_ID)" : "=s"(id));
    asm volatile("s_getreg_b32 %0, hwreg(HW_REG_XCC_ID)" : "=s"(xcc));
    unsigned long long *d = v3_dbg + 3 * ((long long)blockIdx.x * V3_WGW + wv);
    d[0] = (id & 0xffffu) | ((xcc & 0xfu) << 16); d[1] = dbg_t0; d[2] = wall_clock64();
  }
#endif
}

__device__ __forceinline__ long long v3_nchunks(long long total_out, long long grid0, int B) { return total_out > grid0 ? (total_out - grid0 + B - 1) / B : 0; }
__device__ __forceinline__ bool v3_slots_equal(const int *a_, const int *b_)
{
  const int4 *a = reinterpret_cast<const int4 *>(a_), *b = reinterpret_cast<const int4 *>(b_);
  bool same = true;
#pragma unroll
  for (int i = 0; i < 8; i++) { const int4 x = a[i], y = b[i]; same = same && x.x == y.x && x.y == y.y && x.z == y.z && x.w == y.w; }
  return same;
}

__global__ __launch_bounds__(256) void viterbi_check_kernel(V3Aux ax, const RxState *st, long long steps_fixed, VitParams vp, int pass)
{
  const long long total_steps = st ? st->n_vit_steps : steps_fixed;
  const long long nch = v3_nchunks(total_steps / 8 - vp.ntb, ax.grid0, vp.chunk_bytes);
  if (blockIdx.x == 0 && threadIdx.x == 0) { ax.ctl[V3_CTL_CHUNKS] = (int)(nch < INT_MAX ? nch : INT_MAX); if (pass == 1) ax.ctl[V3_CTL_UNPROVEN] = 0; }
  const long long c = (long long)blockIdx.x * 256 + threadIdx.x + 1;
  if (c >= nch || c > ax.cap) return;
  const bool same = v3_slots_equal(v3_own(ax, c), v3_pred(ax, c));
  if (pass == 0) {
    ax.ctl[V3_CTL_HDR + (ax.cap + 2) + c] = 0;
    if (!same) ax.ctl[V3_CTL_HDR + atomicAdd(ax.ctl + V3_CTL_MISMATCH, 1)] = (int)c;
  }
}
__global__ __launch_bounds__(256) void viterbi_count_kernel(V3Aux ax, const RxState *st, long long steps_fixed, VitParams vp)
{
  const long long total_steps = st ? st->n_vit_steps : steps_fixed;
  const long long nch = v3_nchunks(total_steps / 8 - vp.ntb, ax.grid0, vp.chunk_bytes);
  const long long c = (long long)blockIdx.x * 256 + threadIdx.x + 1;
  if (c >= nch || c > ax.cap) return;
  if (!v3_slots_equal(v3_own(ax, c), v3_pred(ax, c))) atomicAdd(ax.ctl + V3_CTL_UNPROVEN, 1);
}

__device__ __forceinline__ bool v3_row_equal(const int (&a)[2], const int (&b)[2], int dd)
{
  const unsigned long long ne = __ballot(a[0] != b[0] || a[1] != b[1]);
  return ((ne >> (16 * dd)) & 0xffffull) == 0;
}

template <int NTB, int NW> __device__ __forceinline__ void v3_repair_rows(const uint8_t *__restrict__ in, uint8_t *__restrict__ out, long long total_steps, const VitParams &vp, const V3Aux &ax,
                                                                  long long in_base, long long out_lo, const V3Lds &S, const V3Lane &L, long long rows, long long row0, int n)
{
  const int lane = threadIdx.x & 63, dd = lane >> 4, pl = lane & 15;
  const long long total_out = total_steps / 8 - vp.ntb;
  const int B = vp.chunk_bytes;
  const long long nch = v3_nchunks(total_out, ax.grid0, B);
  for (long long i0 = row0; i0 < n; i0 += rows) {
    const bool act = i0 + dd < n;
    const long long c = act ? ax.ctl[V3_CTL_HDR + i0 + dd] : 1;
    const long long b0 = ax.grid0 + c * B;
    int v[2], endv[2] = {0, 0};
    { const int *p = v3_pred(ax, c) + 2 * pl; v[0] = p[0]; v[1] = p[1]; }
    int *carry = (act && ax.carry_out && b0 + B >= total_out) ? ax.carry_out + 2 * pl : nullptr;
    v3_decode<NTB, 0, 2, NW>(in, out, total_steps, total_out, vp, in_base, out_lo, b0, act && b0 < total_out, S, L, v, endv, v3_own(ax, c) + 2 * pl, nullptr, nullptr, carry, ax.carry_rel);
    int pn[2] = {endv[0], endv[1]};
    if (act && c + 1 < nch) { const int *p = v3_pred(ax, c + 1) + 2 * pl; pn[0] = p[0]; pn[1] = p[1]; }
    if (!v3_row_equal(endv, pn, dd) || ((ax.debug & 1) && act && c + 1 < nch)) {
      int *f = v3_fix(ax, c + 1) + 2 * pl; f[0] = endv[0]; f[1] = endv[1];
      if (pl == 0) { ax.ctl[V3_CTL_HDR + (ax.cap + 2) + c + 1] = 1; atomicAdd(ax.ctl + V3_CTL_CONFLICT, 1); }
    }
    __builtin_amdgcn_fence(__ATOMIC_SEQ_CST, "wavefront");
  }
}
template <int NTB> __global__ __launch_bounds__(64 * V3_WGW) void viterbi_repair_kernel(const uint8_t *__restrict__ in, uint8_t *__restrict__ out, const RxState *st,
                                                      long long steps_fixed, VitParams vp, V3Aux ax, long long in_base, long long out_lo)
{
  V3_LDS_DECL(V3_WGW)
  const int n = ax.ctl[V3_CTL_MISMATCH];
  const int wv = V3_WGW > 1 ? (int)(threadIdx.x >> 6) : 0;
  const long long rows = (long long)gridDim.x * V3_WGW * 4, row0 = ((long long)blockIdx.x * V3_WGW + wv) * 4;
  if (row0 >= n) return;
  const V3Lds S = V3_LDS(V3_WGW, wv);
  v3_init_lut(sh_.lut, threadIdx.x & 63);
  V3Lane L; v3_init_lane(threadIdx.x & 15, L);
  v3_repair_rows<NTB, V3_WGW>(in, out, st ? st->n_vit_steps : steps_fixed, vp, ax, in_base, out_lo, S, L, rows, row0, n);
}

template <int NTB, int NW> __device__ __forceinline__ void v3_seq_walk(const uint8_t *__restrict__ in, uint8_t *__restrict__ out, long long total_steps, const VitParams &vp, const V3Aux &ax,
                                                               long long in_base, long long out_lo, const V3Lds &S, const V3Lane &L, int force)
{
  const int lane = threadIdx.x & 63, dd = lane >> 4, pl = lane & 15;
  if (lane == 0) { ax.ctl[V3_CTL_ACC] += ax.ctl[V3_CTL_CHUNKS]; ax.ctl[V3_CTL_ACC + 1] += ax.ctl[V3_CTL_MISMATCH]; }
  if (!force && ax.ctl[V3_CTL_CONFLICT] == 0) return;
  const long long total_out = total_steps / 8 - vp.ntb;
  const int B = vp.chunk_bytes;
  long long nch = v3_nchunks(total_out, ax.grid0, B);
  if (nch > ax.cap) nch = ax.cap;
  const int *cflag = ax.ctl + V3_CTL_HDR + (ax.cap + 2);
  int done = 0;
  long long pos = 0;
  for (;;) {
    long long cn = -1;
    for (long long c0 = pos + 1; c0 < nch && cn < 0; c0 += 64) {
      const long long c = c0 + lane;
      bool hit = false;
      if (c < nch) hit = cflag[c] != 0 || (force && !v3_slots_equal(v3_own(ax, c), v3_pred(ax, c)));
      const unsigned long long b = __ballot(hit);
      if (b) cn = c0 + __builtin_ctzll(b);
    }
    if (cn < 0) break;
    long long c = cn;
    int v[2];
    { const int *p = (cflag[c] ? v3_fix(ax, c) : v3_pred(ax, c)) + 2 * pl; v[0] = p[0]; v[1] = p[1]; }
    for (;;) {
      const long long b0 = ax.grid0 + c * B;
      const bool act = dd == 0;
      int st0[2] = {v[0], v[1]}, endv[2] = {0, 0};
      if (act) { int *p = v3_pred(ax, c) + 2 * pl; p[0] = v[0]; p[1] = v[1]; }
      int *carry = (act && ax.carry_out && b0 + B >= total_out) ? ax.carry_out + 2 * pl : nullptr;
      v3_decode<NTB, 0, 2, NW>(in, out, total_steps, total_out, vp, in_base, out_lo, b0, act, S, L, st0, endv, v3_own(ax, c) + 2 * pl, nullptr, nullptr, carry, ax.carry_rel);
      __builtin_amdgcn_fence(__ATOMIC_SEQ_CST, "wavefront");
      done++;
      if (c + 1 >= nch) { pos = nch; break; }
      int on[2]; { const int *p = v3_own(ax, c + 1) + 2 * pl; on[0] = p[0]; on[1] = p[1]; }
      const bool eq = (__ballot(on[0] != endv[0] || on[1] != endv[1]) & 0xffffull) == 0;
      if (act) { int *p = v3_pred(ax, c + 1) + 2 * pl; p[0] = endv[0]; p[1] = endv[1]; }
      if (eq) { pos = c + 1; break; }
      c++; v[0] = endv[0]; v[1] = endv[1];
    }
  }
  if (lane == 0) { ax.ctl[V3_CTL_SEQ] = done; ax.ctl[V3_CTL_ACC + 2] += done; }
}
template <int NTB> __global__ __launch_bounds__(64) void viterbi_repair_seq_kernel(const uint8_t *__restrict__ in, uint8_t *__restrict__ out, const RxState *st,
                                                      long long steps_fixed, VitParams vp, V3Aux ax, long long in_base, long long out_lo, int force)
{
  V3_LDS_DECL(1)
  const V3Lds S = V3_LDS(1, 0);
  v3_init_lut(sh_.lut, threadIdx.x & 63);
  V3Lane L; v3_init_lane(threadIdx.x & 15, L);
  v3_seq_walk<NTB, 1>(in, out, st ? st->n_vit_steps : steps_fixed, vp, ax, in_base, out_lo, S, L, force);
}

constexpr long long V3_FIX_SMALL = 1024;
template <int NTB> __global__ __launch_bounds__(64 * V3_WGW) void viterbi_fix_kernel(const uint8_t *__restrict__ in, uint8_t *__restrict__ out, const RxState *st,
                                                      long long steps_fixed, VitParams vp, V3Aux ax, long long in_base, long long out_lo, int force)
{
  V3_LDS_DECL(V3_WGW)
  const int wv = V3_WGW > 1 ? (int)(threadIdx.x >> 6) : 0;
  const long long total_steps = st ? st->n_vit_steps : steps_fixed;
  const long long nch = v3_nchunks(total_steps / 8 - vp.ntb, ax.grid0, vp.chunk_bytes);
  if (threadIdx.x == 0) ax.ctl[V3_CTL_CHUNKS] = (int)(nch < INT_MAX ? nch : INT_MAX);
  for (long long c = 1 + threadIdx.x; c < nch && c <= ax.cap; c += 64 * V3_WGW) {
    ax.ctl[V3_CTL_HDR + (ax.cap + 2) + c] = 0;
    if (!v3_slots_equal(v3_own(ax, c), v3_pred(ax, c))) ax.ctl[V3_CTL_HDR + atomicAdd(ax.ctl + V3_CTL_MISMATCH, 1)] = (int)c;
  }
  __threadfence(); __syncthreads();
  const int n = *(volatile int *)(ax.ctl + V3_CTL_MISMATCH);
  const V3Lds S = V3_LDS(V3_WGW, wv);
  v3_init_lut(sh_.lut, threadIdx.x & 63);
  V3Lane L; v3_init_lane(threadIdx.x & 15, L);
  if (!force && n > 0) v3_repair_rows<NTB, V3_WGW>(in, out, total_steps, vp, ax, in_base, out_lo, S, L, 4 * V3_WGW, 4 * wv, n);
  __threadfence(); __syncthreads();
  if (wv == 0) v3_seq_walk<NTB, V3_WGW>(in, out, total_steps, vp, ax, in_base, out_lo, S, L, force);
}

}
```

include/dvbt_hip.h:

```cpp
#ifndef DVBT_HIP_H
#define DVBT_HIP_H

#include <stddef.h>
#include <stdint.h>

#ifdef __cplusplus
extern "C" {
#endif

typedef enum {
  DVBT_OK = 0,
  DVBT_ERR_INVALID = -1,
  DVBT_ERR_NO_DEVICE = -2,
  DVBT_ERR_HIP = -3,
  DVBT_ERR_CAPACITY = -4,
  DVBT_ERR_STATE = -5
} dvbt_status;

#ifndef DVBT_HIP_NO_ENUMS
typedef enum { DVBT_QPSK = 0, DVBT_QAM16 = 1, DVBT_QAM64 = 2 } dvbt_constellation_t;
typedef enum { DVBT_NH = 0, DVBT_ALPHA1, DVBT_ALPHA2, DVBT_ALPHA4 } dvbt_hierarchy_t;
typedef enum { DVBT_C1_2 = 0, DVBT_C2_3, DVBT_C3_4, DVBT_C5_6, DVBT_C7_8 } dvbt_code_rate_t;
typedef enum { DVBT_T2k = 0, DVBT_T8k = 1 } dvbt_transmission_mode_t;
typedef enum { DVBT_G1_32 = 0, DVBT_G1_16, DVBT_G1_8, DVBT_G1_4 } dvbt_guard_interval_t;
// ... 27 lines not shown
} dvbt_dims;
int dvbt_get_dims(int constellation, int hierarchy, int code_rate, int guard_interval,
                  int transmission_mode, dvbt_dims *out);

typedef struct { int blocks, fft_length, occupied_tones, cp_length; float snr; } dvbt_ofdm_sym_acquisition_params;
typedef struct dvbt_ofdm_sym_acquisition dvbt_ofdm_sym_acquisition;
int  dvbt_ofdm_sym_acquisition_create(const dvbt_ofdm_sym_acquisition_params *p, dvbt_ofdm_sym_acquisition **out);
int  dvbt_ofdm_sym_acquisition_forecast(const dvbt_ofdm_sym_acquisition *h, int noutput_items, int *ninput_required);
int  dvbt_ofdm_sym_acquisition_work(dvbt_ofdm_sym_acquisition *h, int noutput_items, int ninput_items,
                                    const void *in, void *out, dvbt_sideband *sb);
int  dvbt_ofdm_sym_acquisition_work_device(dvbt_ofdm_sym_acquisition *h, int noutput_items, int ninput_items, const void *in_device, void *out_device,
                                            dvbt_sideband *sb, void *stream);
void dvbt_ofdm_sym_acquisition_destroy(dvbt_ofdm_sym_acquisition *h);

typedef struct { int fft_size; int forward; int shift; } dvbt_fft_params;
typedef struct dvbt_fft dvbt_fft;
int  dvbt_fft_create(const dvbt_fft_params *p, dvbt_fft **out);
int  dvbt_fft_forecast(const dvbt_fft *h, int noutput_items, int *ninput_required);
int  dvbt_fft_work(dvbt_fft *h, int noutput_items, int ninput_items, const void *in, void *out, dvbt_sideband *sb);
int  dvbt_fft_work_device(dvbt_fft *h, int noutput_items, int ninput_items, const void *in_device, void *out_device,
                           dvbt_sideband *sb, void *stream);
void dvbt_fft_destroy(dvbt_fft *h);

typedef struct { int itemsize, ninput, noutput, constellation, hierarchy, code_rate_hp, code_rate_lp,
                 guard_interval, transmission_mode, include_cell_id, cell_id; } dvbt_demod_reference_signals_params;
typedef struct dvbt_demod_reference_signals dvbt_demod_reference_signals;
int  dvbt_demod_reference_signals_create(const dvbt_demod_reference_signals_params *p, dvbt_demod_reference_signals **out);
int  dvbt_demod_reference_signals_forecast(const dvbt_demod_reference_signals *h, int noutput_items, int *ninput_required);
int  dvbt_demod_reference_signals_work(dvbt_demod_reference_signals *h, int noutput_items, int ninput_items,
                                       const void *in, void *out, dvbt_sideband *sb);
int  dvbt_demod_reference_signals_work_device(dvbt_demod_reference_signals *h, int noutput_items, int ninput_items, const void *in_device, void *out_device,
                                               dvbt_sideband *sb, void *stream);
void dvbt_demod_reference_signals_destroy(dvbt_demod_reference_signals *h);

typedef struct { int nsize, constellation, hierarchy, transmission_mode; float gain; } dvbt_demap_params;
typedef struct dvbt_demap dvbt_demap;
int  dvbt_demap_create(const dvbt_demap_params *p, dvbt_demap **out);
int  dvbt_demap_forecast(const dvbt_demap *h, int noutput_items, int *ninput_required);
int  dvbt_demap_work(dvbt_demap *h, int noutput_items, int ninput_items, const void *in, void *out, dvbt_sideband *sb);
int  dvbt_demap_work_device(dvbt_demap *h, int noutput_items, int ninput_items, const void *in_device, void *out_device,
                             dvbt_sideband *sb, void *stream);
void dvbt_demap_destroy(dvbt_demap *h);

typedef struct { int nsize, transmission_mode, direction; } dvbt_symbol_inner_interleaver_params;
typedef struct dvbt_symbol_inner_interleaver dvbt_symbol_inner_interleaver;
int  dvbt_symbol_inner_interleaver_create(const dvbt_symbol_inner_interleaver_params *p, dvbt_symbol_inner_interleaver **out);
int  dvbt_symbol_inner_interleaver_forecast(const dvbt_symbol_inner_interleaver *h, int noutput_items, int *ninput_required);
int  dvbt_symbol_inner_interleaver_work(dvbt_symbol_inner_interleaver *h, int noutput_items, int ninput_items,
                                        const void *in, void *out, dvbt_sideband *sb);
int  dvbt_symbol_inner_interleaver_work_device(dvbt_symbol_inner_interleaver *h, int noutput_items, int ninput_items, const void *in_device, void *out_device,
                                                dvbt_sideband *sb, void *stream);
void dvbt_symbol_inner_interleaver_destroy(dvbt_symbol_inner_interleaver *h);

typedef struct { int nsize, constellation, hierarchy, transmission_mode; } dvbt_bit_inner_deinterleaver_params;
typedef struct dvbt_bit_inner_deinterleaver dvbt_bit_inner_deinterleaver;
int  dvbt_bit_inner_deinterleaver_create(const dvbt_bit_inner_deinterleaver_params *p, dvbt_bit_inner_deinterleaver **out);
int  dvbt_bit_inner_deinterleaver_forecast(const dvbt_bit_inner_deinterleaver *h, int noutput_items, int *ninput_required);
int  dvbt_bit_inner_deinterleaver_work(dvbt_bit_inner_deinterleaver *h, int noutput_items, int ninput_items,
                                       const void *in, void *out, dvbt_sideband *sb);
int  dvbt_bit_inner_deinterleaver_work_device(dvbt_bit_inner_deinterleaver *h, int noutput_items, int ninput_items, const void *in_device, void *out_device,
                                               dvbt_sideband *sb, void *stream);
int  dvbt_bit_inner_deinterleaver_work_hier(dvbt_bit_inner_deinterleaver *h, int noutput_items, int ninput_items,
                                            const void *in, void *out_hp, void *out_lp, dvbt_sideband *sb);
int  dvbt_bit_inner_deinterleaver_work_hier_device(dvbt_bit_inner_deinterleaver *h, int noutput_items, int ninput_items, const void *in_device,
                                                   void *out_hp_device, void *out_lp_device, dvbt_sideband *sb, void *stream);
void dvbt_bit_inner_deinterleaver_destroy(dvbt_bit_inner_deinterleaver *h);

typedef struct {
  int64_t chunks;
  int64_t decoded_again;
  int64_t sequential;
  int64_t not_proven;
} dvbt_viterbi_proof;
typedef struct { int constellation, hierarchy, code_rate, bsize, S0, SK; } dvbt_viterbi_decoder_params;
typedef struct dvbt_viterbi_decoder dvbt_viterbi_decoder;
int  dvbt_viterbi_decoder_create(const dvbt_viterbi_decoder_params *p, dvbt_viterbi_decoder **out);
int  dvbt_viterbi_decoder_forecast(const dvbt_viterbi_decoder *h, int noutput_items, int *ninput_required);
int  dvbt_viterbi_decoder_work(dvbt_viterbi_decoder *h, int noutput_items, int ninput_items,
                               const void *in, void *out, dvbt_sideband *sb);
int  dvbt_viterbi_decoder_work_device(dvbt_viterbi_decoder *h, int noutput_items, int ninput_items, const void *in_device, void *out_device,
                                       dvbt_sideband *sb, void *stream);
int  dvbt_viterbi_decoder_set_warm_windows(dvbt_viterbi_decoder *h, int windows);
int  dvbt_viterbi_decoder_proof(dvbt_viterbi_decoder *h, dvbt_viterbi_proof *out);
void dvbt_viterbi_decoder_destroy(dvbt_viterbi_decoder *h);

typedef struct { int blocks, I, M; } dvbt_convolutional_deinterleaver_params;
typedef struct dvbt_convolutional_deinterleaver dvbt_convolutional_deinterleaver;
int  dvbt_convolutional_deinterleaver_create(const dvbt_convolutional_deinterleaver_params *p, dvbt_convolutional_deinterleaver **out);
int  dvbt_convolutional_deinterleaver_forecast(const dvbt_convolutional_deinterleaver *h, int noutput_items, int *ninput_required);
int  dvbt_convolutional_deinterleaver_work(dvbt_convolutional_deinterleaver *h, int noutput_items, int ninput_items,
                                           const void *in, void *out, dvbt_sideband *sb);
int  dvbt_convolutional_deinterleaver_work_device(dvbt_convolutional_deinterleaver *h, int noutput_items, int ninput_items, const void *in_device, void *out_device,
                                                   dvbt_sideband *sb, void *stream);
void dvbt_convolutional_deinterleaver_destroy(dvbt_convolutional_deinterleaver *h);

typedef struct { int p, m, gfpoly, n, k, t, s, blocks; int oracle_compat; } dvbt_reed_solomon_dec_params;
typedef struct dvbt_reed_solomon_dec dvbt_reed_solomon_dec;
int  dvbt_reed_solomon_dec_create(const dvbt_reed_solomon_dec_params *p, dvbt_reed_solomon_dec **out);
int  dvbt_reed_solomon_dec_forecast(const dvbt_reed_solomon_dec *h, int noutput_items, int *ninput_required);
int  dvbt_reed_solomon_dec_work(dvbt_reed_solomon_dec *h, int noutput_items, int ninput_items,
                                const void *in, void *out, dvbt_sideband *sb);
int  dvbt_reed_solomon_dec_work_device(dvbt_reed_solomon_dec *h, int noutput_items, int ninput_items, const void *in_device, void *out_device,
                                        dvbt_sideband *sb, void *stream);
void dvbt_reed_solomon_dec_destroy(dvbt_reed_solomon_dec *h);

typedef struct { int nblocks; } dvbt_energy_descramble_params;
typedef struct dvbt_energy_descramble dvbt_energy_descramble;
int  dvbt_energy_descramble_create(const dvbt_energy_descramble_params *p, dvbt_energy_descramble **out);
int  dvbt_energy_descramble_forecast(const dvbt_energy_descramble *h, int noutput_items, int *ninput_required);
int  dvbt_energy_descramble_work(dvbt_energy_descramble *h, int noutput_items, int ninput_items,
                                 const void *in, void *out, dvbt_sideband *sb);
int  dvbt_energy_descramble_work_device(dvbt_energy_descramble *h, int noutput_items, int ninput_items, const void *in_device, void *out_device,
                                         dvbt_sideband *sb, void *stream);
void dvbt_energy_descramble_destroy(dvbt_energy_descramble *h);

typedef struct { int interpolation, decimation; float scale; } dvbt_resampler_params;
typedef struct dvbt_resampler dvbt_resampler;
int  dvbt_resampler_create(const dvbt_resampler_params *p, dvbt_resampler **out);
int  dvbt_resampler_forecast(const dvbt_resampler *h, int noutput_items, int *ninput_required);
int  dvbt_resampler_work(dvbt_resampler *h, int noutput_items, int ninput_items,
                         const void *in, void *out, dvbt_sideband *sb);
int  dvbt_resampler_work_device(dvbt_resampler *h, int noutput_items, int ninput_items, const void *in_device, void *out_device,
                                dvbt_sideband *sb, void *stream);
int  dvbt_resampler_get_taps(const dvbt_resampler *h, float *taps, int cap, int *interpolation, int *decimation);
void dvbt_resampler_destroy(dvbt_resampler *h);


typedef struct { int nblocks; } dvbt_energy_dispersal_params;
typedef struct dvbt_energy_dispersal dvbt_energy_dispersal;
int  dvbt_energy_dispersal_create(const dvbt_energy_dispersal_params *p, dvbt_energy_dispersal **out);
int  dvbt_energy_dispersal_forecast(const dvbt_energy_dispersal *h, int noutput_items, int *ninput_required);
int  dvbt_energy_dispersal_work(dvbt_energy_dispersal *h, int noutput_items, int ninput_items, const void *in, void *out, dvbt_sideband *sb);
int  dvbt_energy_dispersal_work_device(dvbt_energy_dispersal *h, int noutput_items, int ninput_items, const void *in_device, void *out_device,
                                       dvbt_sideband *sb, void *stream);
void dvbt_energy_dispersal_destroy(dvbt_energy_dispersal *h);

typedef struct { int p, m, gfpoly, n, k, t, s, blocks; } dvbt_reed_solomon_enc_params;
typedef struct dvbt_reed_solomon_enc dvbt_reed_solomon_enc;
int  dvbt_reed_solomon_enc_create(const dvbt_reed_solomon_enc_params *p, dvbt_reed_solomon_enc **out);
int  dvbt_reed_solomon_enc_forecast(const dvbt_reed_solomon_enc *h, int noutput_items, int *ninput_required);
int  dvbt_reed_solomon_enc_work(dvbt_reed_solomon_enc *h, int noutput_items, int ninput_items, const void *in, void *out, dvbt_sideband *sb);
int  dvbt_reed_solomon_enc_work_device(dvbt_reed_solomon_enc *h, int noutput_items, int ninput_items, const void *in_device, void *out_device,
                                       dvbt_sideband *sb, void *stream);
void dvbt_reed_solomon_enc_destroy(dvbt_reed_solomon_enc *h);

typedef struct { int blocks, I, M; } dvbt_convolutional_interleaver_params;
typedef struct dvbt_convolutional_interleaver dvbt_convolutional_interleaver;
int  dvbt_convolutional_interleaver_create(const dvbt_convolutional_interleaver_params *p, dvbt_convolutional_interleaver **out);
int  dvbt_convolutional_interleaver_forecast(const dvbt_convolutional_interleaver *h, int noutput_items, int *ninput_required);
int  dvbt_convolutional_interleaver_work(dvbt_convolutional_interleaver *h, int noutput_items, int ninput_items, const void *in, void *out, dvbt_sideband *sb);
int  dvbt_convolutional_interleaver_work_device(dvbt_convolutional_interleaver *h, int noutput_items, int ninput_items, const void *in_device, void *out_device,
                                                dvbt_sideband *sb, void *stream);
void dvbt_convolutional_interleaver_destroy(dvbt_convolutional_interleaver *h);

typedef struct { int ninput, noutput, constellation, hierarchy, code_rate; } dvbt_inner_coder_params;
typedef struct dvbt_inner_coder dvbt_inner_coder;
int  dvbt_inner_coder_create(const dvbt_inner_coder_params *p, dvbt_inner_coder **out);
int  dvbt_inner_coder_forecast(const dvbt_inner_coder *h, int noutput_items, int *ninput_required);
int  dvbt_inner_coder_work(dvbt_inner_coder *h, int noutput_items, int ninput_items, const void *in, void *out, dvbt_sideband *sb);
int  dvbt_inner_coder_work_device(dvbt_inner_coder *h, int noutput_items, int ninput_items, const void *in_device, void *out_device,
                                  dvbt_sideband *sb, void *stream);
void dvbt_inner_coder_destroy(dvbt_inner_coder *h);

typedef struct { int nsize, constellation, hierarchy, transmission_mode; } dvbt_bit_inner_interleaver_params;
typedef struct dvbt_bit_inner_interleaver dvbt_bit_inner_interleaver;
int  dvbt_bit_inner_interleaver_create(const dvbt_bit_inner_interleaver_params *p, dvbt_bit_inner_interleaver **out);
// ... 28 lines not shown
  int viterbi_bsize;
  int rs_oracle_compat;
  int descramble;
  size_t max_samples;
  int device;
  int viterbi_chunk_bytes;
  int resample_interp, resample_decim;
  float front_scale;
  int soft_decision;
  int hier_stream;
  int launch_graph;
  int front_priority;
  int viterbi_warm_windows;
  int viterbi_verify;
} dvbt_rx_params;

typedef struct {
  int32_t status;
  int32_t n_symbols;
  int32_t first_out_symbol;
  int32_t n_out_symbols;
  int32_t cp_start0;
  int32_t first_call;
  int64_t n_viterbi_bytes;
  int64_t n_rs_items;
  int64_t n_rs_bytes;
  int64_t n_ts_bytes;
  int32_t rs_fail_words, rs_corrected_symbols;
  int64_t resume_sample;
  int64_t segment_offset;
  int64_t stream_symbol_offset;
  int64_t ts_first_packet;
  int64_t stream_rs_items;
  uint64_t tps_bits;
  int32_t tps_valid;
  int32_t tps_length_indicator, tps_constellation, tps_hierarchy, tps_code_rate_hp, tps_code_rate_lp,
          tps_guard_interval, tps_transmission_mode, tps_cell_id;
  int32_t tps_mismatch;
  int32_t n_lock_periods;
  int32_t total_symbols;
} dvbt_rx_report;

typedef enum {
  DVBT_TAP_ACQ = 0,
  DVBT_TAP_FFT = 1,
  DVBT_TAP_EQ = 2,
  DVBT_TAP_DEMAP = 3,
  DVBT_TAP_SYMDEINT = 4,
  DVBT_TAP_BITDEINT = 5,
  DVBT_TAP_VITERBI = 6,
  DVBT_TAP_DEINT = 7,
  DVBT_TAP_RS = 8,
  DVBT_TAP_TS = 9,
  DVBT_TAP_CP_START = 10,
  DVBT_TAP_SYMBOL_INDEX = 11,
  DVBT_TAP_FREQ_OFFSET = 12,
  DVBT_TAP_BITDEINT_LP = 13,
  DVBT_TAP_SOFT = 14,
  DVBT_TAP_BITDEINT_LOG = 16,
  DVBT_TAP_CSI = 15
} dvbt_tap;

typedef struct dvbt_rx dvbt_rx;
int  dvbt_rx_create(const dvbt_rx_params *p, dvbt_rx **out);
typedef struct {
  int64_t stream_symbol_offset;
  int32_t start_delay_symbols;
  int32_t descr_call_phase;
} dvbt_rx_cut;
int  dvbt_rx_set_cut(dvbt_rx *h, const dvbt_rx_cut *cut);
int  dvbt_rx_segment_run(dvbt_rx *h, const void *iq_host, size_t nsamples, dvbt_rx_report *report);
int  dvbt_rx_segment_run_device(dvbt_rx *h, const void *iq_device, size_t nsamples, void *stream, dvbt_rx_report *report);
int  dvbt_rx_segment_enqueue_device(dvbt_rx *h, const void *iq_device, size_t nsamples, void *stream);
int  dvbt_rx_segment_finish(dvbt_rx *h, dvbt_rx_report *report);
typedef struct {
  int64_t offset;
  int32_t first_call;
  int32_t cp_start0;
  int32_t n_symbols;
  int32_t first_out_symbol;
} dvbt_lock_period;
int  dvbt_rx_viterbi_proof(dvbt_rx *h, dvbt_viterbi_proof *out);
int  dvbt_rx_viterbi_proof_total(dvbt_rx *h, dvbt_viterbi_proof *out);
int  dvbt_rx_viterbi_check(dvbt_rx *h, int64_t *chunks, int64_t *unproven);
int  dvbt_rx_lock_periods(dvbt_rx *h, dvbt_lock_period *out, int cap);
typedef struct { int64_t small_passes, general_passes; int32_t small_chunk_calls, small_max_calls; } dvbt_walk_stats;
int  dvbt_rx_walk_stats(dvbt_rx *h, dvbt_walk_stats *out);
int64_t dvbt_rx_read_tap(dvbt_rx *h, int tap, void *dst_host, size_t cap_bytes);
void *dvbt_rx_tap_device_ptr(dvbt_rx *h, int tap);
double dvbt_rx_stage_ms(dvbt_rx *h, const char *stage);
int  dvbt_rx_enable_timing(dvbt_rx *h, int enable);
int  dvbt_rx_enable_taps(dvbt_rx *h, int enable);
typedef struct { int64_t bitdeint_offset, bitdeint_bytes, viterbi_offset, viterbi_bytes; } dvbt_period_tap;
int  dvbt_rx_period_taps(dvbt_rx *h, dvbt_period_tap *out, int cap);
typedef struct {
  int64_t mer_carriers;  double mer_signal, mer_error;
  int64_t channel_bits, channel_bit_errors;
  int64_t post_bits, post_bit_errors;
  int32_t rs_fail_words, rs_corrected_symbols, n_lock_periods, flags;
} dvbt_rx_quality_report;
int  dvbt_rx_enable_quality(dvbt_rx *h, int enable);
int  dvbt_rx_quality(dvbt_rx *h, dvbt_rx_quality_report *out);
void dvbt_rx_destroy(dvbt_rx *h);

typedef struct {
  dvbt_rx_params rx; int segment_superframes;
  int rank, world;
  int64_t ts_ring_bytes;
  int borrow_device_pushes;
  int chains;
} dvbt_rx_stream_params;
typedef struct {
  int32_t status;
  int32_t pieces_in_flight, finished;
  int64_t samples_pushed, ts_bytes_decoded, ts_bytes_ready, ts_bytes_pulled;
  int64_t first_superframe_call;
  int64_t first_ts_packet;
  int32_t constellation, hierarchy, code_rate;
  int32_t auto_configured;
  int64_t samples_released;
  int32_t in_walk;
} dvbt_rx_stream_info;
typedef struct dvbt_rx_stream dvbt_rx_stream;
int  dvbt_rx_stream_create(const dvbt_rx_stream_params *p, dvbt_rx_stream **out);
int  dvbt_rx_stream_push(dvbt_rx_stream *s, const void *iq_host, size_t nsamples);
int  dvbt_rx_stream_push_device(dvbt_rx_stream *s, const void *iq_device, size_t nsamples, void *stream);
int64_t dvbt_rx_stream_pull(dvbt_rx_stream *s, void *ts_host, size_t cap);
int64_t dvbt_rx_stream_pull_chunk(dvbt_rx_stream *s, void *ts_host, size_t cap, int64_t *first_packet);
int  dvbt_rx_stream_finish(dvbt_rx_stream *s);
int  dvbt_rx_stream_status(const dvbt_rx_stream *s, dvbt_rx_stream_info *info);
int64_t dvbt_rx_stream_trace(const dvbt_rx_stream *s, char *dst, size_t cap);
int  dvbt_rx_stream_viterbi_proof(const dvbt_rx_stream *s, dvbt_viterbi_proof *out);
void dvbt_rx_stream_destroy(dvbt_rx_stream *s);

typedef struct dvbt_rccl_comm dvbt_rccl_comm;
int  dvbt_rccl_unique_id(void *id128_out);
int  dvbt_rccl_comm_create(const void *id128, int rank, int world, int device, dvbt_rccl_comm **out);
void dvbt_rccl_comm_destroy(dvbt_rccl_comm *c);
typedef struct { int64_t first_packet; int64_t nbytes; int64_t offset; } dvbt_gather_chunk;
int  dvbt_rx_stream_set_device_output(dvbt_rx_stream *s, size_t ring_bytes);
int  dvbt_rx_stream_gather_enqueue(dvbt_rx_stream *s, dvbt_rccl_comm *c, int root, int slot_packets);
int64_t dvbt_rx_stream_gather_wait(dvbt_rx_stream *s, dvbt_rccl_comm *c, void *ts_host, size_t cap, dvbt_gather_chunk *chunks, int *all_done);
const void *dvbt_rccl_step_buffer(const dvbt_rccl_comm *c);
#define DVBT_GATHER_DEVICE 1
int  dvbt_rx_stream_gather_enqueue_ex(dvbt_rx_stream *s, dvbt_rccl_comm *c, int root, int slot_packets, int flags);
const void *dvbt_rccl_step_device_buffer(const dvbt_rccl_comm *c);
int  dvbt_rccl_comm_reserve(dvbt_rccl_comm *c, int root, int slot_packets, int flags);
int64_t dvbt_rx_stream_gather(dvbt_rx_stream *s, dvbt_rccl_comm *c, int root, int slot_packets, void *ts_host, size_t cap, dvbt_gather_chunk *chunks, int *all_done);

typedef struct {
  int constellation, hierarchy, code_rate, guard_interval, transmission_mode, include_cell_id, cell_id;
  float scale;
  size_t max_packets;
  int64_t first_packet;
  int keep_carriers;
  int device;
} dvbt_tx_params;
typedef struct dvbt_tx dvbt_tx;
int     dvbt_tx_create(const dvbt_tx_params *p, dvbt_tx **out);
int64_t dvbt_tx_samples_for(const dvbt_tx *h, size_t npackets);
int     dvbt_tx_run(dvbt_tx *h, const void *ts_host, size_t npackets, void *iq_host, size_t cap_samples, size_t *nsamples);
int     dvbt_tx_run_device(dvbt_tx *h, const void *ts_device, size_t npackets, void *iq_device, size_t cap_samples, void *stream, size_t *nsamples);
int64_t dvbt_tx_read_carriers(dvbt_tx *h, void *dst_host, size_t cap_bytes);
int     dvbt_tx_reset(dvbt_tx *h);
void    dvbt_tx_destroy(dvbt_tx *h);

// ... 68 lines not shown
```

Before: 37550.

## Skip Viterbi traceback walk when consecutive survivor links agree with best states

```diff
diff --git a/gr_dvbt_amd/binding.py b/gr_dvbt_amd/binding.py
--- a/gr_dvbt_amd/binding.py
+++ b/gr_dvbt_amd/binding.py
@@ -271,6 +271,16 @@
         _chk(self.L.dvbt_rx_viterbi_proof_total(self.h, C.byref(p)))
         return {"chunks": int(p.chunks), "decoded_again": int(p.decoded_again), "sequential": int(p.sequential), "not_proven": int(p.not_proven)}
 
+    def set_viterbi_walk(self, always):
+        self.L.dvbt_rx_set_viterbi_walk.argtypes = [C.c_void_p, C.c_int]
+        _chk(self.L.dvbt_rx_set_viterbi_walk(self.h, int(bool(always))))
+
+    def viterbi_shortcut(self):
+        out = (C.c_longlong * 2)()
+        self.L.dvbt_rx_viterbi_shortcut.argtypes = [C.c_void_p, C.POINTER(C.c_longlong)]
+        _chk(self.L.dvbt_rx_viterbi_shortcut(self.h, out))
+        return int(out[0]), int(out[1])
+
     def viterbi_check(self):
         a, b = C.c_int64(), C.c_int64()
         self.L.dvbt_rx_viterbi_check.argtypes = [C.c_void_p, C.POINTER(C.c_int64), C.POINTER(C.c_int64)]
@@ -628,6 +638,16 @@
         _chk(self.L.dvbt_viterbi_decoder_proof(self.h, C.byref(p)))
         return {"chunks": int(p.chunks), "decoded_again": int(p.decoded_again), "sequential": int(p.sequential), "not_proven": int(p.not_proven)}
 
+    def set_viterbi_walk(self, always):
+        self.L.dvbt_viterbi_decoder_set_walk.argtypes = [C.c_void_p, C.c_int]
+        _chk(self.L.dvbt_viterbi_decoder_set_walk(self.h, int(bool(always))))
+
+    def viterbi_shortcut(self):
+        out = (C.c_longlong * 2)()
+        self.L.dvbt_viterbi_decoder_shortcut.argtypes = [C.c_void_p, C.POINTER(C.c_longlong)]
+        _chk(self.L.dvbt_viterbi_decoder_shortcut(self.h, out))
+        return int(out[0]), int(out[1])
+
     def close(self):
         if self.h:
             fn = getattr(self.L, f"dvbt_{self.name}_destroy")
diff --git a/gr_dvbt_amd/csrc/dvbt_blocks.inc b/gr_dvbt_amd/csrc/dvbt_blocks.inc
--- a/gr_dvbt_amd/csrc/dvbt_blocks.inc
+++ b/gr_dvbt_amd/csrc/dvbt_blocks.inc
@@ -299,6 +299,7 @@
   dvbt_viterbi_decoder_params p; BlockCtx c; Dims d; VitParams vp;
   size_t hist = 0; long long in_total = 0, steps = 0; int d_init = 0;
   static constexpr size_t kTail = 8192;
+  bool walk = false;
   VitProof proof; DevMem<int> carry; int cur = 0; bool have_carry = false; long long grid0 = 0;
 };
 extern "C" int dvbt_viterbi_decoder_create(const dvbt_viterbi_decoder_params *p, dvbt_viterbi_decoder **out)
@@ -342,13 +343,13 @@
     if (!dev) { WCHK(h->c.dout.reserve((size_t)produced)); o = (uint8_t *)h->c.dout.p; }
     const int B = h->vp.chunk_bytes;
     const long long g0 = h->have_carry ? h->grid0 : 0, chunks = (out_hi - g0 + B - 1) / B;
-    if (chunks + 2 > h->proof.cap) { HIPCHK(hipStreamSynchronize(s)); int acc[3]; HIPCHK(hipMemcpy(acc, h->proof.ctl + V3_CTL_ACC, sizeof acc, hipMemcpyDeviceToHost));
+    if (chunks + 2 > h->proof.cap) { HIPCHK(hipStreamSynchronize(s)); int acc[8]; HIPCHK(hipMemcpy(acc, h->proof.ctl + V3_CTL_ACC, sizeof acc, hipMemcpyDeviceToHost));
                                      WCHK(h->proof.reserve(2 * chunks + 2)); HIPCHK(hipMemcpy(h->proof.ctl + V3_CTL_ACC, acc, sizeof acc, hipMemcpyHostToDevice)); }
     V3Aux ax = h->proof.aux();
     ax.grid0 = g0; ax.carry_in = h->have_carry ? h->carry + h->cur * V3_SLOT : nullptr;
     const long long b0_last = g0 + (chunks - 1) * B;
     ax.carry_rel = (int)((out_hi - b0_last) / V3_BLK) * V3_BLK; ax.carry_out = h->carry + (h->cur ^ 1) * V3_SLOT;
-    launch_viterbi(s, (const uint8_t *)h->c.din.p, o, (const RxState *)nullptr, h->steps, h->vp, in_base, out_lo, produced, &ax, VIT_REPAIR);
+    launch_viterbi(s, (const uint8_t *)h->c.din.p, o, (const RxState *)nullptr, h->steps, h->vp, in_base, out_lo, produced, &ax, VIT_REPAIR, h->walk);
     h->cur ^= 1; h->have_carry = true; h->grid0 = b0_last + ax.carry_rel;
     if (!dev) WCHK(h->c.get(out, h->c.dout.p, (size_t)produced));
   }
@@ -390,6 +391,18 @@
   int acc[3] = {0, 0, 0};
   HIPCHK(hipMemcpy(acc, h->proof.ctl + V3_CTL_ACC, sizeof acc, hipMemcpyDeviceToHost));
   out->chunks = acc[0]; out->decoded_again = acc[1]; out->sequential = acc[2]; out->not_proven = -1;
+  return DVBT_OK;
+}
+extern "C" int dvbt_viterbi_decoder_set_walk(dvbt_viterbi_decoder *h, int always)
+{
+  if (!h) return fail(DVBT_ERR_INVALID, "null handle");
+  h->walk = always != 0;
+  return DVBT_OK;
+}
+extern "C" int dvbt_viterbi_decoder_shortcut(dvbt_viterbi_decoder *h, long long out[2])
+{
+  if (!h || !out) return fail(DVBT_ERR_INVALID, "null argument");
+  HIPCHK(hipMemcpy(out, h->proof.ctl + V3_CTL_SHORT, 2 * sizeof(long long), hipMemcpyDeviceToHost));
   return DVBT_OK;
 }
 extern "C" void dvbt_viterbi_decoder_destroy(dvbt_viterbi_decoder *h) { delete h; }
diff --git a/gr_dvbt_amd/csrc/dvbt_hip.hip b/gr_dvbt_amd/csrc/dvbt_hip.hip
--- a/gr_dvbt_amd/csrc/dvbt_hip.hip
+++ b/gr_dvbt_amd/csrc/dvbt_hip.hip
@@ -203,7 +203,7 @@
 constexpr unsigned V3_REPAIR_GRID = 64;
 
 static void launch_viterbi(hipStream_t s, const uint8_t *in, uint8_t *out, const RxState *st, long long steps_fixed, const VitParams &vp,
-                           long long in_base, long long out_lo, long long max_out_bytes, const V3Aux *ax = nullptr, int mode = VIT_PLAIN)
+                           long long in_base, long long out_lo, long long max_out_bytes, const V3Aux *ax = nullptr, int mode = VIT_PLAIN, bool walk = false)
 {
   const bool proof = ax && mode != VIT_PLAIN;
   const long long grid0 = proof ? ax->grid0 : out_lo;
@@ -211,9 +211,11 @@
   if (chunks < 1) chunks = 1;
   const dim3 grid((unsigned)((chunks + 4 * V3_WGW - 1) / (4 * V3_WGW))), blk(64 * V3_WGW);
   V3Aux none; memset(&none, 0, sizeof none);
+  if (walk) none.debug |= V3_DEBUG_WALK;
   if (proof) {
     V3Aux a = *ax;
-    if (mode == VIT_FORCE_CONFLICT) { a.debug = 1; mode = VIT_REPAIR_COUNT; }
+    if (walk) a.debug |= V3_DEBUG_WALK;
+    if (mode == VIT_FORCE_CONFLICT) { a.debug |= 1; mode = VIT_REPAIR_COUNT; }
     const dim3 cgrid((unsigned)((chunks + 255) / 256));
     if (vp.warm == V3_WARM) {
 #define V3_CALL(N) hipLaunchKernelGGL((viterbi3_kernel<N, V3_WARM, 1>), grid, blk, 0, s, in, out, st, steps_fixed, vp, a, in_base, out_lo)
@@ -344,6 +346,7 @@
   DevMem<float2> q_sym; DevMem<double> q_mer; DevMem<unsigned long long> q_cnt;
   unsigned long long seg_serial = 0, q_eq_serial = 0;
   DevMem<uint8_t> bd_log; std::vector<dvbt_period_tap> plog; size_t plog_bytes = 0;
+  bool vit_walk = false;
   VitProof vproof; bool vit_checked = false;
   size_t vit_cap = 0; DevMem<RsDefer> rs_defer; int rs_defer_cap = 0;
   DevMem<unsigned long long> rs_sync;
@@ -764,7 +767,7 @@
     h->vit_checked = true;
   }
   launch_viterbi(s, (const uint8_t *)((h->prm.hier_stream && h->bitdeint_lp) ? h->bitdeint_lp : h->bitdeint), h->vit + o.vit_off, (const RxState *)h->st, 0ll, vp, 0ll, 0ll, max_vit,
-                 proof ? &ax : nullptr, h->prm.viterbi_verify);
+                 proof ? &ax : nullptr, h->prm.viterbi_verify, h->vit_walk);
   }
   if (tmv) HIPCHK(hipEventRecord(h->ev[ST_RS], s));
   if (o.tail) { int r = enqueue_tail(h, s, max_vit / 204 + 1, -1); if (r) return r; }
@@ -1350,6 +1353,23 @@
   out->chunks = acc[0]; out->decoded_again = acc[1]; out->sequential = acc[2]; out->not_proven = -1;
   return DVBT_OK;
 }
+extern "C" int dvbt_rx_set_viterbi_walk(dvbt_rx *h, int always)
+{
+  if (!h) return fail(DVBT_ERR_INVALID, "null handle");
+  if (h->pending) return fail(DVBT_ERR_STATE, "dvbt_rx_set_viterbi_walk: a segment is in flight (dvbt_rx_segment_finish first)");
+  h->vit_walk = always != 0;
+  drop_graphs(h);
+  return DVBT_OK;
+}
+extern "C" int dvbt_rx_viterbi_shortcut(dvbt_rx *h, long long out[2])
+{
+  if (!h || !out) return fail(DVBT_ERR_INVALID, "null argument");
+  if (!h->vproof.ctl) return fail(DVBT_ERR_STATE, "dvbt_rx_viterbi_shortcut: the handle runs the plain chunk decoders (viterbi_verify = -1, or soft decisions)");
+  if (h->pending) return fail(DVBT_ERR_STATE, "dvbt_rx_viterbi_shortcut: a segment is in flight (dvbt_rx_segment_finish first)");
+  HIPCHK(hipSetDevice(h->prm.device));
+  HIPCHK(hipMemcpy(out, h->vproof.ctl + V3_CTL_SHORT, 2 * sizeof(long long), hipMemcpyDeviceToHost));
+  return DVBT_OK;
+}
 extern "C" int dvbt_rx_viterbi_check(dvbt_rx *h, int64_t *chunks, int64_t *unproven)
 {
   if (!h || !chunks || !unproven) return fail(DVBT_ERR_INVALID, "null argument");
diff --git a/gr_dvbt_amd/csrc/k_viterbi3.hpp b/gr_dvbt_amd/csrc/k_viterbi3.hpp
--- a/gr_dvbt_amd/csrc/k_viterbi3.hpp
+++ b/gr_dvbt_amd/csrc/k_viterbi3.hpp
@@ -261,6 +261,7 @@
 constexpr int V3_CTL_UNPROVEN = 3;
 constexpr int V3_CTL_SEQ = 4;
 constexpr int V3_CTL_ACC = 8;
+constexpr int V3_CTL_SHORT = 12;
 constexpr int V3_CTL_HDR = 16;
 struct V3Aux {
   int *snap;
@@ -271,6 +272,7 @@
   int *carry_out; int carry_rel;
   int debug;
 };
+constexpr int V3_DEBUG_WALK = 2;
 __device__ __forceinline__ int *v3_own(const V3Aux &ax, long long c) { return ax.snap + (3 * c) * V3_SLOT; }
 __device__ __forceinline__ int *v3_pred(const V3Aux &ax, long long c) { return ax.snap + (3 * c + 1) * V3_SLOT; }
 __device__ __forceinline__ int *v3_fix(const V3Aux &ax, long long c) { return ax.snap + (3 * c + 2) * V3_SLOT; }
@@ -292,7 +294,7 @@
 template <int NTB, int WARM, int MODE, int NW>
 __device__ __forceinline__ void v3_decode(const uint8_t *__restrict__ in, uint8_t *__restrict__ out, long long total_steps, long long total_out, const VitParams &vp,
                                           long long in_base, long long out_lo, long long b0, bool dec_active, const V3Lds &S, const V3Lane &L, int (&v)[2], int (&endv)[2],
-                                          int *own, int *predn, const int *inject, int *carry, int carry_rel)
+                                          int *own, int *predn, const int *inject, int *carry, int carry_rel, int debug, unsigned long long *shortcut)
 {
   unsigned char *const tab = S.tab; unsigned *const wbuf = S.wbuf; unsigned char *const bests = S.bests; const unsigned *const lut = S.lut;
   unsigned *const cbits = wbuf;
@@ -362,7 +364,7 @@
       }
     }
   };
-  auto stage_words = [&](int jb) {
+  auto stage_words = [&](int jb, auto &&mid) {
     {
       const unsigned mk = (1u << m) - 1;
       auto grp = [&](unsigned d) { return ((d & mk) << (3 * m)) | (((d >> 8) & mk) << (2 * m)) | (((d >> 16) & mk) << m) | ((d >> 24) & mk); };
@@ -396,6 +398,7 @@
     const unsigned kmask = ((unsigned)(vp.punct_rep >> ph) << (2 * lo)) & (((1u << (2 * hi)) - 1u) & ~((1u << (2 * lo)) - 1u));
     const unsigned *cb = cbits + dd * V3_CBS;
     const unsigned cw0 = cb[pos >> 5], cw1 = cb[(pos >> 5) + 1];
+    mid();
     unsigned win = (unsigned)(((((unsigned long long)cw0) << 32) | cw1) >> (32 - (pos & 31)));
     unsigned idx[SPL], sw[SPL];
 #pragma unroll
@@ -414,8 +417,10 @@
   };
   V3Trace T;
   int tsh[2];
+  int tsh_e[2];
 #pragma unroll
   for (int c = 0; c < 2; c++) {
+    tsh_e[c] = (2 * ((c * 16 + pl + 1 + 3 * ntb - (ntb - 1)) % 3) + 4) % 6;
     T.oend[c] = c * 16 + pl < V3_BLK ? ob_end : INT_MIN; tsh[c] = (2 * ((c * 16 + pl + 1) % 3) + 4) % 6; T.osh[c] = (6 - 2 * ((c * 16 + pl + 3 * ntb - (ntb - 1)) % 3)) % 6;
   }
   static_assert(V3_BLK % 3 == 0, "phases per lane");
@@ -423,6 +428,7 @@
 #pragma unroll
     for (int c = 0; c < 2; c++) bb[c] = bests[dd * V3_RINGW + ((jp + c * 16 + pl) & (V3_RINGW - 1))];
   };
+  auto z_of_best = [](unsigned b, int sh) { const unsigned R = (b | (b << 6)) >> sh; return (R ^ 51u ^ (((R >> 4) & 1u) * 12u)) & 63u; };
   auto trace_init = [&](int jp, const unsigned (&bb)[2]) {
 #pragma unroll
     for (int c = 0; c < 2; c++) {
@@ -430,11 +436,33 @@
       T.ob[c] = jj - (warm + ntb - 1);
       T.ok[c] = __builtin_amdgcn_ballot_w64(T.ob[c] >= ob_lo && T.ob[c] < T.oend[c]);
       T.wsh[c] = jj * V3_ROW<NW> + rowl;
-      const unsigned R = (bb[c] | (bb[c] << 6)) >> tsh[c];
-      T.z[c] = (int)((R ^ 51u ^ (((R >> 4) & 1u) * 12u)) & 63u) | (T.wsh[c] & V3_RMASK<NW>);
+      T.z[c] = (int)z_of_best(bb[c], tsh[c]) | (T.wsh[c] & V3_RMASK<NW>);
     }
   };
-  unsigned bb[2];
+  unsigned bb[2], be[2], tl[2], te[2];
+  int zp[2], zcarry = 0;
+  auto bests_read_ends = [&](int jp) {
+#pragma unroll
+    for (int c = 0; c < 2; c++) be[c] = bests[dd * V3_RINGW + ((jp + c * 16 + pl - (ntb - 1)) & (V3_RINGW - 1))];
+  };
+  auto link_reads = [&](int jp) {
+    trace_init(jp, bb);
+    zp[0] = __builtin_amdgcn_update_dpp(zcarry, T.z[0], 0x111, 0xf, 0xf, false);
+    zp[1] = __builtin_amdgcn_update_dpp(dppb<0x121>(T.z[0]), T.z[1], 0x111, 0xf, 0xf, false);
+#pragma unroll
+    for (int c = 0; c < 2; c++) tl[c] = tab[T.z[c]];
+    zcarry = dppb<0x129>(T.z[1]);
+  };
+  auto end_reads = [&]() {
+#pragma unroll
+    for (int c = 0; c < 2; c++) te[c] = tab[(int)z_of_best(be[c], tsh_e[c]) | ((T.wsh[c] - (ntb - 1) * V3_ROW<NW>) & V3_RMASK<NW>)];
+  };
+  auto links_hold = [&](int jp) {
+    const bool fails = jp - (warm + ntb - 1) < ob_end && ((((tl[0] ^ (unsigned)zp[0]) & 63u) != 0) || (pl < V3_BLK - 16 && ((tl[1] ^ (unsigned)zp[1]) & 63u) != 0));
+    return __builtin_amdgcn_ballot_w64(fails) == 0;
+  };
+  bool ok_prev = false;
+  unsigned n_short = 0, n_walk = 0;
 
   stage_load(0);
   for (int jb = 0; jb < J; jb += V3_BLK) {
@@ -449,10 +477,17 @@
       if (carry && dec_active && jb == carry_rel) { carry[0] = v[0]; carry[1] = v[1]; }
     }
     bests_read(jb - V3_BLK, bb);
-    if (!(V3_EXP & 8) || jb == 0) stage_words(jb);
+    bests_read_ends(jb - V3_BLK);
+    if (!(V3_EXP & 8) || jb == 0) stage_words(jb, [&]() { link_reads(jb - V3_BLK); });
+    else link_reads(jb - V3_BLK);
     if (jb + V3_BLK < J && !(V3_EXP & 8)) stage_load(jb + V3_BLK);
-    const bool tr = jb > 0 && !(V3_EXP & 1);
-    if (tr) trace_init(jb - V3_BLK, bb);
+    const bool ok_cur = jb > 0 && links_hold(jb - V3_BLK);
+    const bool ends = (T.ok[0] | T.ok[1]) != 0;
+    const bool fast = ok_cur && ok_prev && !(debug & V3_DEBUG_WALK) && !(V3_EXP & 1);
+    ok_prev = ok_cur;
+    const bool tr = jb > 0 && !fast && ends && !(V3_EXP & 1);
+    if (fast && ends) { end_reads(); v3_trace_store<true>(T, te, outb); n_short++; }
+    if (tr) n_walk++;
     const unsigned *wrow = wbuf + dd * (V3_BLK * 8);
     unsigned Wa[8], Wb[8];
     v3_load_words(wrow, Wa);
@@ -473,6 +508,7 @@
   trace_init(J - V3_BLK, bb);
   for (int h = 0; h < ntb - 1; h++) v3_hop<NW>(T, tab);
   v3_trace_out(T, tab, outb);
+  if (MODE == 1 && shortcut && lane == 0) { atomicAdd(shortcut, (unsigned long long)n_short); atomicAdd(shortcut + 1, (unsigned long long)n_walk); }
 }
 
 template <int NW> struct V3Shared {
@@ -515,7 +551,8 @@
     if (c == 0 && ax.carry_in) inject = ax.carry_in + 2 * pl;
     if (ax.carry_out && b0 + B >= total_out) carry = ax.carry_out + 2 * pl;
   }
-  v3_decode<NTB, WARM, MODE, V3_WGW>(in, out, total_steps, total_out, vp, in_base, out_lo, b0, dec_active, S, L, v, endv, own, predn, inject, carry, ax.carry_rel);
+  v3_decode<NTB, WARM, MODE, V3_WGW>(in, out, total_steps, total_out, vp, in_base, out_lo, b0, dec_active, S, L, v, endv, own, predn, inject, carry, ax.carry_rel, ax.debug,
+                                     MODE == 1 ? reinterpret_cast<unsigned long long *>(ax.ctl + V3_CTL_SHORT) : nullptr);
 #if V3_EXP & 16
   if (lane == 0) {
     unsigned id, xcc;
@@ -579,7 +616,7 @@
     int v[2], endv[2] = {0, 0};
     { const int *p = v3_pred(ax, c) + 2 * pl; v[0] = p[0]; v[1] = p[1]; }
     int *carry = (act && ax.carry_out && b0 + B >= total_out) ? ax.carry_out + 2 * pl : nullptr;
-    v3_decode<NTB, 0, 2, NW>(in, out, total_steps, total_out, vp, in_base, out_lo, b0, act && b0 < total_out, S, L, v, endv, v3_own(ax, c) + 2 * pl, nullptr, nullptr, carry, ax.carry_rel);
+    v3_decode<NTB, 0, 2, NW>(in, out, total_steps, total_out, vp, in_base, out_lo, b0, act && b0 < total_out, S, L, v, endv, v3_own(ax, c) + 2 * pl, nullptr, nullptr, carry, ax.carry_rel, ax.debug, nullptr);
     int pn[2] = {endv[0], endv[1]};
     if (act && c + 1 < nch) { const int *p = v3_pred(ax, c + 1) + 2 * pl; pn[0] = p[0]; pn[1] = p[1]; }
     if (!v3_row_equal(endv, pn, dd) || ((ax.debug & 1) && act && c + 1 < nch)) {
@@ -635,7 +672,7 @@
       int st0[2] = {v[0], v[1]}, endv[2] = {0, 0};
       if (act) { int *p = v3_pred(ax, c) + 2 * pl; p[0] = v[0]; p[1] = v[1]; }
       int *carry = (act && ax.carry_out && b0 + B >= total_out) ? ax.carry_out + 2 * pl : nullptr;
-      v3_decode<NTB, 0, 2, NW>(in, out, total_steps, total_out, vp, in_base, out_lo, b0, act, S, L, st0, endv, v3_own(ax, c) + 2 * pl, nullptr, nullptr, carry, ax.carry_rel);
+      v3_decode<NTB, 0, 2, NW>(in, out, total_steps, total_out, vp, in_base, out_lo, b0, act, S, L, st0, endv, v3_own(ax, c) + 2 * pl, nullptr, nullptr, carry, ax.carry_rel, ax.debug, nullptr);
       __builtin_amdgcn_fence(__ATOMIC_SEQ_CST, "wavefront");
       done++;
       if (c + 1 >= nch) { pos = nch; break; }
diff --git a/include/dvbt_hip.h b/include/dvbt_hip.h
--- a/include/dvbt_hip.h
+++ b/include/dvbt_hip.h
@@ -133,6 +133,8 @@
                                        dvbt_sideband *sb, void *stream);
 int  dvbt_viterbi_decoder_set_warm_windows(dvbt_viterbi_decoder *h, int windows);
 int  dvbt_viterbi_decoder_proof(dvbt_viterbi_decoder *h, dvbt_viterbi_proof *out);
+int  dvbt_viterbi_decoder_set_walk(dvbt_viterbi_decoder *h, int always);
+int  dvbt_viterbi_decoder_shortcut(dvbt_viterbi_decoder *h, long long out[2]);
 void dvbt_viterbi_decoder_destroy(dvbt_viterbi_decoder *h);
 
 typedef struct { int blocks, I, M; } dvbt_convolutional_deinterleaver_params;
@@ -327,6 +329,8 @@
 } dvbt_lock_period;
 int  dvbt_rx_viterbi_proof(dvbt_rx *h, dvbt_viterbi_proof *out);
 int  dvbt_rx_viterbi_proof_total(dvbt_rx *h, dvbt_viterbi_proof *out);
+int  dvbt_rx_set_viterbi_walk(dvbt_rx *h, int always);
+int  dvbt_rx_viterbi_shortcut(dvbt_rx *h, long long out[2]);
 int  dvbt_rx_viterbi_check(dvbt_rx *h, int64_t *chunks, int64_t *unproven);
 int  dvbt_rx_lock_periods(dvbt_rx *h, dvbt_lock_period *out, int cap);
 typedef struct { int64_t small_passes, general_passes; int32_t small_chunk_calls, small_max_calls; } dvbt_walk_stats;
```

Result: faster. 38320 (median of 6 runs) (+2.1%).
